# supersimple33/aruco-slam

Measured on AMD Instinct MI355X. Metric: EKF updates/sec at n=1024 landmarks, m=32 obs/frame, higher is better.
Workload: dtype f32 covariance / f64 state

## Files before the change

aruco_slam_amd/_build.py:

```python
from __future__ import annotations

import os
import shutil
import subprocess
from pathlib import Path

PKG = Path(__file__).resolve().parent
CSRC = PKG / "csrc"
LIB_DIR = PKG / "lib"
LIB_PATH = LIB_DIR / "libekf_slam_hip.so"
SOURCES = ["ekf_api.hip", "ekf_batch_api.hip", "ekf_small_kernels.hip", "ekf_front.hip", "ekf_front_f64.hip", "ekf_cov_update.hip", "ekf_cov_macro.hip", "ekf_cov_strip.hip", "ekf_pose_ippe.hip",
           "ekf_wide.hip", "ekf_log.hip", "ekf_gate.hip", "ekf_remove.hip", "ekf_motion.hip", "ekf_batch.hip", "ekf_batch_rot.hip", "ekf_batch_wide.hip", "ekf_batch_moved.hip", "ekf_batch_wide_moved.hip",
           "ekf_batch_frozen.hip", "ekf_batch_wide_frozen.hip",
           "ekf_batch_replicas.hip", "ekf_batch_corner_replicas.hip", "ekf_smooth.hip"]
HEADERS = ["ekf_device.h", "ekf_kernels.h", "ekf_solve_device.h", "ekf_solve_big.h", "ekf_solve_cw.h", "ekf_front_impl.h", "ekf_markers.h", "ekf_host.h", "ekf_batch_impl.h", "ekf_gate_device.h", "ekf_motion_device.h", "ekf_ippe_device.h", "ekf_philox.h", "ekf_remove.h", "ekf_smooth_device.h",
           "../../include/ekf_slam_hip.h"]


def hipcc() -> str:
    for cand in (os.environ.get("HIPCC"), shutil.which("hipcc"), "/opt/rocm/bin/hipcc"):
        if cand and Path(cand).exists():
            return cand
    raise RuntimeError("hipcc not found (need /opt/rocm)")


def _stale(target: Path, deps) -> bool:
    if not target.exists():
        return True
    t = target.stat().st_mtime
    return any(Path(d).stat().st_mtime > t for d in deps)


def build(force: bool = False, verbose: bool = False) -> Path:
    LIB_DIR.mkdir(exist_ok=True)
    obj_dir = PKG / "build"
    obj_dir.mkdir(exist_ok=True)
    hdrs = [CSRC / h for h in HEADERS]
    objs = []
    flags = ["--offload-arch=gfx950", "-O3", "-fPIC", "-std=c++17", "-Wall", "-Wno-unused-function"]
    jobs = []
    for src in SOURCES:
        obj = obj_dir / (Path(src).stem + ".o")
        if force or _stale(obj, [CSRC / src, *hdrs]):
            jobs.append([hipcc(), *flags, "-c", str(CSRC / src), "-o", str(obj)])
        objs.append(obj)
    if jobs:
        from concurrent.futures import ThreadPoolExecutor
        def run(cmd):
            if verbose:
                print(" ".join(cmd))
            subprocess.run(cmd, check=True)
        with ThreadPoolExecutor(max_workers=min(6, len(jobs))) as pool:
            list(pool.map(run, jobs))
    if force or _stale(LIB_PATH, objs):
        cmd = [hipcc(), "--offload-arch=gfx950", "-shared", "-fPIC", "-o", str(LIB_PATH),
               *map(str, objs)]
        if verbose:
            print(" ".join(cmd))
        subprocess.run(cmd, check=True)
    return LIB_PATH


if __name__ == "__main__":
    print(build(verbose=True))
```

aruco_slam_amd/csrc/ekf_api.hip:

```cpp
#include <atomic>
#include <cmath>
#include <cstring>

#include "ekf_host.h"
#include "ekf_kernels.h"
#include "ekf_remove.h"

thread_local std::string g_err;

namespace {

std::atomic<ekf_filter*> g_pipelining{nullptr};

void release_pipelining_token(ekf_filter* f) { (void)g_pipelining.compare_exchange_strong(f, nullptr); }

constexpr int kStageSlots = 64;
constexpr int kMacroSuper = 8;
constexpr int kMacroMinTiles = 3000;
constexpr int kTimedKernels = 4;
constexpr int kWideVisible = 1024;
inline int visible_cap(int model) { return model == EKF_MODEL_ROTATIONS ? 50 : 64; }
inline bool wide_frame(int model, int m) { return m > visible_cap(model); }
constexpr int kEventPool = 2048;

// ... 57 lines not shown
        const size_t nb = (size_t)L.kmax / EKF_RB;
        L.xl_dop = nb * (nb - 1) / 2 * 256 + 64;
        L.xl_y = L.xl_dop + nb * 256;
        L.xl_jac = L.xl_y + L.kmax;
        L.xl_tag = L.xl_jac + (size_t)L.kmax * EKF_JLD;
        L.xl_xs = L.xl_tag + 32;
        L.xl_xr = L.xl_xs + nb * (nb + 1) / 2 * 256;
        L.xl_stag = L.xl_xr + (size_t)round_up(L.kmax, 16);
        L.xl_len = L.xl_stag + 256;
        L.off_xl = w.take(2 * L.xl_len * 8);
        L.off_done = w.take(256);
        L.off_sync = w.take(EKF_SYNC_WORDS * 8);
        L.wsup_ld = (int)round_up(EKF_CAM + (int64_t)L.lmd * c.max_visible, 32);
        L.off_wsup = w.take((size_t)2 * L.kmax * L.wsup_ld * L.elem);
    }
    {
        const int tmax = (int)(L.cap / 128);
        L.tiles_cap = (L.elem == 4 && c.cov_kernel != EKF_COVK_VALU && c.cov_kernel != EKF_COVK_MFMA_TILE)
                          ? tmax * (tmax + 1) / 2 + 8 * kMacroSuper * kMacroSuper : 0;
        L.off_tiles = w.take((size_t)L.tiles_cap * 4);
    }
    L.off_wwork = wide ? w.take((size_t)L.kmax * L.cap * 8) : 0;
    L.off_xinv = wide ? w.take((size_t)EKF_WIDE_BLOCK * EKF_WIDE_BLOCK * 8) : 0;
    L.has_gate = (c.flags & EKF_FLAG_GATE) != 0;
    L.off_gidx = L.has_gate ? w.take((size_t)c.max_visible * 4) : 0;
    L.off_gz = L.has_gate ? w.take((size_t)c.max_visible * 7 * 8) : 0;
    L.off_gmahal = L.has_gate ? w.take((size_t)c.max_visible * 8) : 0;
    L.has_rows = (c.flags & EKF_FLAG_ROW_NOISE) != 0;
    L.off_grow = L.has_rows && L.has_gate ? w.take((size_t)c.max_visible * L.rd * 8) : 0;
    L.total = w.end;
    const size_t det_bytes = align256((size_t)c.max_visible * 4) + align256((size_t)c.max_visible * 56);
    L.slot_exempt = det_bytes;
    L.slot_mahal = det_bytes + align256((size_t)c.max_visible);
    L.slot_rows = L.has_gate ? L.slot_mahal + align256((size_t)c.max_visible * 8) : det_bytes;
    L.slot_bytes = std::max(L.has_rows ? L.slot_rows + align256((size_t)c.max_visible * L.rd * 8) : L.slot_rows,
                            align256(256 * 48) + align256(256 * 80));
    return L;
}

int check_config(const ekf_config* c) {
    if (!c) return fail(EKF_ERR_INVALID, "config is NULL");
    if (c->max_landmarks < 1) return fail(EKF_ERR_INVALID, "max_landmarks must be >= 1");
    if (c->model != EKF_MODEL_EKF && c->model != EKF_MODEL_ROTATIONS)
        return fail(EKF_ERR_INVALID, "unknown model");
    if (c->max_visible < 1 || c->max_visible > ((c->flags & EKF_FLAG_WIDE_FRAMES) ? kWideVisible : visible_cap(c->model)))
        return fail(EKF_ERR_INVALID, (c->flags & EKF_FLAG_WIDE_FRAMES)
                                         ? "max_visible must be in 1..1024 (EKF_FLAG_WIDE_FRAMES)"
                                         : "max_visible must be in 1..64 (1..50 for EKF_MODEL_ROTATIONS; up to 1024 with "
                                           "EKF_FLAG_WIDE_FRAMES)");
    if (c->cov_dtype != EKF_COV_F64 && c->cov_dtype != EKF_COV_F32)
        return fail(EKF_ERR_INVALID, "cov_dtype must be EKF_COV_F64 or EKF_COV_F32");
    if (c->quat_mode != EKF_QUAT_AS_WRITTEN && c->quat_mode != EKF_QUAT_SCALAR_FIRST)
        return fail(EKF_ERR_INVALID, "unknown quat_mode");
    if (c->cov_kernel < EKF_COVK_AUTO || c->cov_kernel > EKF_COVK_MFMA_MACRO)
        return fail(EKF_ERR_INVALID, "unknown cov_kernel");
    if (c->cov_kernel == EKF_COVK_MFMA_MACRO && c->cov_dtype != EKF_COV_F32)
        return fail(EKF_ERR_INVALID, "EKF_COVK_MFMA_MACRO exists for the f32 covariance only");
    if (!(c->r_uncertainty > 0.0)) return fail(EKF_ERR_INVALID, "r_uncertainty must be > 0");
    return EKF_OK;
}

}

struct GetterShortcut {
    bool front_pending = false, mirror_fresh = false, mirror_trust = false, status_clean = false;
    bool zero_copy() const { return mirror_fresh && mirror_trust && status_clean; }
    void frame(bool recorded, bool mirrored) { front_pending = recorded; mirror_fresh = mirrored; }
    void run() { front_pending = status_clean = false; }
    void log() { front_pending = mirror_fresh = false; }
    void markers_added() { front_pending = false; }
    void state_set() { front_pending = mirror_trust = false; }
    void reset() { *this = {false, false, true, true}; }
    void new_workspace() { *this = {}; }
    void removed() { front_pending = mirror_fresh = false; mirror_trust = true; }
    void moved() { front_pending = mirror_fresh = false; }
    void read_back(bool clean, bool full_state) { status_clean = clean; mirror_trust = mirror_trust || full_state; }
};

struct ekf_filter {
    ekf_config cfg{};
    Layout lay{};
    hipStream_t stream = nullptr;
    hipStream_t big = nullptr;
    hipEvent_t ev_front = nullptr;
    GetterShortcut shortcut;
    int device = 0;
    void* cov = nullptr;
    int64_t ld = 0;
    double* state = nullptr;
    char* ws = nullptr;
    bool bound = false, is_reset = false;
    int n_lm = 0;
    int last_m = 0;
    bool debug_w = false;
    bool debug_stamps = false;
    bool debug_stamps_light = false;
    uint64_t fseq = 0;
    uint64_t done_total = 0;
    uint64_t la_base = 0;
    int la_ok = -1;
    int seq_mode = EKF_SEQ_NONE;
    int tiles_T = -1, tiles_grid = 0;
    PinnedBuffer ring, readback, tiles_host;
    int slot = 0;
    hipEvent_t slot_done[kStageSlots] = {};
    bool timing = false;
    bool timing_cov_only = false;
    std::vector<hipEvent_t> ev;
    int ev_frames = 0;
    double t_sum_us[kTimedKernels] = {};
    int64_t t_cnt[kTimedKernels] = {};
    PinnedBuffer log_pin[2];
    hipEvent_t log_pin_done[2] = {};
    int log_pin_turn = 0;
    int64_t log_stats[4] = {};
    double gate = __builtin_inf();
    PinnedBuffer gate_pin;
    hipEvent_t ev_gate = nullptr;
    int64_t gate_stats[2] = {};
    PinnedBuffer remove_pin[2];
    hipEvent_t remove_done[2] = {};
    int remove_turn = 0;

    double pending = 0.0;

    bool frozen = false;

    struct HistoryRec {
        int32_t frame, dims;
        size_t off;
        double s_eff;
        double u[6];
        int32_t stepped, moved;
    };
    struct History {
        bool valid = false;
        const void* buf = nullptr;
        size_t bytes = 0;
        int32_t frames = 0;
        std::vector<HistoryRec> recs;
        std::vector<int32_t> frame_rec;
        std::vector<EkfSmoothRec> table;
    } hist;

    bool has_scale() const { return (cfg.flags & EKF_FLAG_FRAME_SCALE) != 0; }
    bool has_motion() const { return (cfg.flags & EKF_FLAG_MOTION) != 0; }
    bool gate_on() const { return lay.has_gate && gate < __builtin_inf(); }
    void reset_gate_stats() { gate_stats[0] = gate_stats[1] = 0; }
    int dims() const { return lay.lmd * n_lm + EKF_CAM; }
    template <typename P> P* at(size_t off) const { return reinterpret_cast<P*>(ws + off); }
};

namespace {

template <class F>
auto by_cov_type(const ekf_filter* f, F&& fn) {
    return f->lay.elem == 4 ? fn(float{}) : fn(double{});
}

int fold_timing(ekf_filter* f) {
    if (f->ev_frames == 0) return EKF_OK;
    HIP_TRY(hipStreamSynchronize(f->stream));
    for (int fr = 0; fr < f->ev_frames; ++fr) {
        for (int kq = f->timing_cov_only ? kTimedKernels - 1 : 0; kq < kTimedKernels; ++kq) {
            float ms = 0.f;
            HIP_TRY(hipEventElapsedTime(&ms, f->ev[fr * (kTimedKernels + 1) + kq],
                                        f->ev[fr * (kTimedKernels + 1) + kq + 1]));
            f->t_sum_us[kq] += 1e3 * ms;
            f->t_cnt[kq] += 1;
        }
    }
    f->ev_frames = 0;
    return EKF_OK;
}

EkfNoise frame_noise(const ekf_filter* f, double s_eff) {
    return EkfNoise{s_eff * f->cfg.q_cam, s_eff * f->cfg.q_err, s_eff * f->cfg.q_lm, f->cfg.r_uncertainty};
}

bool scale_ok(double s) { return std::isfinite(s) && s >= 0.0; }

EkfFrame make_frame(ekf_filter* f, const int32_t* idx_dev, const double* z_dev, const double* rows_dev, int m,
                    double* traj_row, double s_eff) {
    EkfFrame fr{};
// ... 4 lines not shown
    fr.model = f->cfg.model;
    fr.dims = f->dims();
    fr.ncols = (int)round_up(fr.dims, 128);
    fr.m = m;
    fr.k = L.rd * m;
    fr.kpad = (int)round_up(fr.k, EKF_RB);
    fr.idx = idx_dev;
    fr.z = z_dev;
    fr.rrow = rows_dev;
    fr.jac = f->at<double>(L.off_jac);
    fr.resid = f->at<double>(L.off_resid);
    fr.lmcol = f->at<int32_t>(L.off_lmcol);
    fr.amat = f->at<double>(L.off_amat);
    fr.lda = L.cap;
    fr.sblk = f->at<double>(L.off_sblk);
    fr.lmat = f->at<double>(L.off_lmat);
    fr.ldl = L.kmax;
    fr.dinv = f->at<double>(L.off_dinv);
    fr.lop = f->at<double>(L.off_lop);
    fr.dop = f->at<double>(L.off_dop);
    fr.yvec = f->at<double>(L.off_y);
    fr.wpanel = f->at<void>(L.off_wpanel);
    fr.ldw = L.cap;
    fr.wdbg = f->debug_w ? f->at<double>(L.off_wdbg) : nullptr;
    fr.status = f->at<int32_t>(L.off_status);
    fr.traj_row = traj_row;
    fr.dxvec = f->at<double>(L.off_dx);
    fr.stamps = (f->debug_w || f->debug_stamps) ? f->at<long long>(L.off_stamps) : nullptr;
    fr.stamps_heavy = f->debug_stamps_light ? 0 : 1;
    fr.gate_log = (fr.stamps && !fr.stamps_heavy && !f->debug_w && (size_t)L.kmax * L.cap >= 4 * EKF_GATE_LOG_FRAMES)
                      ? f->at<long long>(L.off_wdbg) : nullptr;
    fr.nz = frame_noise(f, s_eff);
    fr.qprev_cam = fr.nz.q_cam;
    fr.qprev_err = fr.nz.q_err;
    fr.qprev_lm = fr.nz.q_lm;
    fr.quat_mode = f->cfg.quat_mode;
    fr.n_lm = f->n_lm;
    fr.state_host = nullptr;
    fr.status_host = nullptr;
    fr.frozen = f->frozen ? 1 : 0;
    fr.cov_tiles = nullptr;
    fr.cov_grid = 0;
    if (f->tiles_T > 0 && f->tiles_T == (fr.dims + 127) / 128) {
        fr.cov_tiles = f->at<uint32_t>(L.off_tiles);
        fr.cov_grid = f->tiles_grid;
    }
    return fr;
}

bool use_front_kernel(const ekf_filter* f, const EkfFrame& fr) { return (f->cfg.flags & 4) == 0 && fr.kpad <= 192; }

void bind_exchange(ekf_filter* f, EkfFrame& fr) {
    const Layout& L = f->lay;
    double* base = f->at<double>(L.off_xl);
    fr.xl = base + (f->fseq & 1) * L.xl_len;
    fr.xl_next = base + ((f->fseq + 1) & 1) * L.xl_len;
    fr.xl_dop = (int32_t)L.xl_dop;
    fr.xl_y = (int32_t)L.xl_y;
    fr.xl_jac = (int32_t)L.xl_jac;
    fr.xl_tag = (int32_t)L.xl_tag;
    fr.xl_len = (int32_t)L.xl_len;
    fr.xs = fr.xl + L.xl_xs;
    fr.xr = fr.xl + L.xl_xr;
    fr.xs_tag = fr.xl + L.xl_stag;
    fr.seqno = (double)(f->fseq + 1);
    fr.done_ctr = f->at<unsigned long long>(L.off_done);
    f->done_total += (uint64_t)(fr.ncols / 64);
    fr.done_target = f->done_total;
    f->fseq++;
}

int ensure_tiles(ekf_filter* f) {
    const Layout& L = f->lay;
    const int T = (f->dims() + 127) / 128;
    const bool want = L.tiles_cap > 0 &&
                      (f->cfg.cov_kernel == EKF_COVK_MFMA_MACRO || T * (T + 1) / 2 >= kMacroMinTiles);
    if (!want) {
        f->tiles_T = -1;
        return EKF_OK;
    }
    if (f->tiles_T == T) return EKF_OK;
    HIP_TRY(hipStreamSynchronize(f->stream));
    HIP_TRY(hipStreamSynchronize(f->big));
    const int grid = ekf_cov_macro_table(T, kMacroSuper, f->tiles_host.at<uint32_t>(0), L.tiles_cap);
    if (grid <= 0) return fail(EKF_ERR_STATE, "macro-tile launch table does not fit the workspace");
    HIP_TRY(hipMemcpy(f->at<uint32_t>(L.off_tiles), f->tiles_host.get(), (size_t)grid * 4, hipMemcpyHostToDevice));
    f->tiles_T = T;
    f->tiles_grid = grid;
    return EKF_OK;
}

int enqueue_frame(ekf_filter* f, const int32_t* idx_dev, const double* z_dev, const double* rows_dev, int m,
                  double* traj_row, bool mirror, double s_eff) {
    if (!f->frozen) {
        int trc = ensure_tiles(f);
        if (trc) return trc;
    }
    EkfFrame fr = make_frame(f, idx_dev, z_dev, rows_dev, m, traj_row, s_eff);
    const int variant = f->cfg.cov_kernel == EKF_COVK_VALU ? 1 : 2;
    hipEvent_t* ev = nullptr;
    if (f->timing) {
        if (f->ev_frames == kEventPool) {
            int rc = fold_timing(f);
            if (rc) return rc;
        }
        ev = &f->ev[f->ev_frames * (kTimedKernels + 1)];
        f->ev_frames++;
    }
    hipEvent_t* ev_all = (ev && !f->timing_cov_only) ? ev : nullptr;
    if (ev_all) HIP_TRY(hipEventRecord(ev[0], f->stream));
    const bool mirrored = use_front_kernel(f, fr) && !f->timing && mirror && !f->frozen;
    if (use_front_kernel(f, fr)) {
        bind_exchange(f, fr);
        if (mirrored) {
            fr.state_host = f->readback.at<double>(256);
            fr.status_host = f->readback.at<int32_t>(128);
        }
        by_cov_type(f, [&](auto elem) { ekf_launch_front<decltype(elem)>(fr, f->stream); });
        if (ev_all) {
            HIP_TRY(hipEventRecord(ev[1], f->stream));
            HIP_TRY(hipEventRecord(ev[2], f->stream));
        }
    } else if (wide_frame(fr.model, m)) {
        const bool blocked = fr.kpad > EKF_WIDE_REUSE_ROWS;
        const int rp = blocked ? (int)round_up(fr.k, EKF_WIDE_BLOCK) : fr.kpad;
        double* aw = blocked ? f->at<double>(f->lay.off_wwork) : nullptr;
        if (blocked && !f->lay.off_wwork) return fail(EKF_ERR_STATE, "internal: no wide-frame workspace");
        by_cov_type(f, [&](auto elem) { ekf_launch_wide_front<decltype(elem)>(fr, aw, rp, f->stream); });
        if (ev_all) HIP_TRY(hipEventRecord(ev[1], f->stream));
        if (blocked) ekf_launch_wide_factor(fr, aw, f->at<double>(f->lay.off_xinv), rp, f->stream);
        else ekf_launch_solve(fr, f->stream);
        if (ev_all) HIP_TRY(hipEventRecord(ev[2], f->stream));
        by_cov_type(f, [&](auto elem) {
            if (blocked) ekf_launch_wide_finish<decltype(elem)>(fr, aw, f->stream);
            else ekf_launch_panel<decltype(elem)>(fr, f->stream);
        });
        if (fr.model == 1) ekf_launch_inject_rot(fr, f->frozen ? 0 : f->n_lm, f->stream);
    } else {
        by_cov_type(f, [&](auto elem) { ekf_launch_gather<decltype(elem)>(fr, f->stream); });
        if (ev_all) HIP_TRY(hipEventRecord(ev[1], f->stream));
        ekf_launch_solve(fr, f->stream);
        if (ev_all) HIP_TRY(hipEventRecord(ev[2], f->stream));
        by_cov_type(f, [&](auto elem) { ekf_launch_panel<decltype(elem)>(fr, f->stream); });
        if (fr.model == 1) ekf_launch_inject_rot(fr, f->frozen ? 0 : f->n_lm, f->stream);
    }
    f->shortcut.frame(!f->timing && hipEventRecord(f->ev_front, f->stream) == hipSuccess, mirrored);
    if (fr.kpad > EKF_WIDE_REUSE_ROWS) {
        if (ev) HIP_TRY(hipEventRecord(ev[3], f->stream));
        for (int r0 = 0; r0 < fr.kpad; r0 += EKF_WIDE_REUSE_ROWS) {
            EkfFrame cf = fr;
            cf.wpanel = static_cast<char*>(fr.wpanel) + (size_t)r0 * fr.ldw * f->lay.elem;
            cf.kpad = std::min(EKF_WIDE_REUSE_ROWS, fr.kpad - r0);
            cf.k = std::min(cf.kpad, std::max(0, fr.k - r0));
            if (r0 > 0) cf.nz.q_cam = cf.nz.q_err = cf.nz.q_lm = 0.0;
            const bool ok = by_cov_type(f, [&](auto elem) {
                if (f->frozen) return ekf_launch_cov_strip<decltype(elem)>(cf, variant, f->stream);
                ekf_launch_cov_update<decltype(elem)>(cf, variant, f->stream);
                return true;
            });
            if (!ok) return fail(EKF_ERR_STATE, "internal: a row chunk larger than the strip kernel takes");
        }
        if (ev) HIP_TRY(hipEventRecord(ev[4], f->stream));
    } else {
        const bool ok = by_cov_type(f, [&](auto elem) {
            if (f->frozen) return ekf_launch_cov_strip<decltype(elem)>(fr, variant, f->stream, ev ? ev[3] : nullptr, ev ? ev[4] : nullptr);
            ekf_launch_cov_update<decltype(elem)>(fr, variant, f->stream, ev ? ev[3] : nullptr, ev ? ev[4] : nullptr);
            return true;
        });
        if (!ok) return fail(EKF_ERR_STATE, "internal: more rows than the strip kernel takes in one launch");
    }
    HIP_TRY(hipGetLastError());
    f->last_m = m;
    return EKF_OK;
}

int check_ready(ekf_filter* f) {
    if (!f) return fail(EKF_ERR_INVALID, "filter handle is NULL");
    if (!f->bound) return fail(EKF_ERR_STATE, "ekf_bind_buffers has not been called");
    if (!f->is_reset) return fail(EKF_ERR_STATE, "ekf_reset has not been called");
    HIP_TRY(hipSetDevice(f->device));
    return EKF_OK;
}

int sync_and_check(ekf_filter* f, int state_count = 0) {
    if (state_count > 0 && f->shortcut.front_pending) {
        HIP_TRY(hipEventSynchronize(f->ev_front));
        if (f->shortcut.zero_copy() && *f->readback.at<volatile int32_t>(128) == 0)
            return EKF_OK;
        HIP_TRY(hipMemcpyAsync(f->readback.get(), f->at<int32_t>(f->lay.off_status), 32, hipMemcpyDeviceToHost, f->big));
        HIP_TRY(hipMemcpyAsync(f->readback.at<double>(256), f->state, (size_t)state_count * 8, hipMemcpyDeviceToHost, f->big));
        HIP_TRY(hipStreamSynchronize(f->big));
    } else {
        HIP_TRY(hipMemcpyAsync(f->readback.get(), f->at<int32_t>(f->lay.off_status), 32, hipMemcpyDeviceToHost, f->stream));
        if (state_count > 0)
            HIP_TRY(hipMemcpyAsync(f->readback.at<double>(256), f->state, (size_t)state_count * 8, hipMemcpyDeviceToHost, f->stream));
        HIP_TRY(hipStreamSynchronize(f->stream));
        release_pipelining_token(f);
    }
    const int32_t* info = f->readback.at<int32_t>(0);
    const int32_t st = info[0];
    f->shortcut.read_back(st == 0, state_count == f->dims());
    if (st != 0) {
        if (st & EKF_ST_BAD_INDEX)
            return fail(EKF_ERR_INVALID, "landmark index out of range in a device-resident detection array "
                                         "(clamped on the device; the filter state is no longer meaningful, reset it)");
        if (st & (EKF_ST_STALE_JAC | EKF_ST_STALE_COL | EKF_ST_STALE_S))
            return fail(EKF_ERR_NUMERIC, "internal: exchange data of another frame accepted in the front kernel (status " +
                                             std::to_string(st) + ")");
        if (st & EKF_ST_GATE_TIMEOUT)
            return fail(EKF_ERR_NUMERIC, "internal: a device-side wait between the two streams of the pipelined sequence mode timed out");
        if (st & EKF_ST_TIMEOUT)
            return fail(EKF_ERR_NUMERIC, "internal: exchange wait timed out in the front kernel (status " +
                                             std::to_string(st) + ")");
        if (info[2] >= 200)
            return fail(EKF_ERR_NUMERIC, "internal: a wait inside the factorisation workgroup timed out (flag word " +
                                             std::to_string(info[2] - 200) + ")");
        return fail(EKF_ERR_NUMERIC, "innovation covariance S was not positive definite (block column " +
                                         std::to_string(info[2] - 100) + ", wave mask " + std::to_string(info[1]) + ")");
    }
    return EKF_OK;
}

bool pipeline_wanted(const ekf_filter* f, int dims, int kpad, int m) {
    const bool auto_on = !(dims > 9000 && kpad > 96) && !(f->cfg.model == EKF_MODEL_ROTATIONS && kpad > 64);
    const bool want = (f->cfg.flags & 2) != 0 || ((f->cfg.flags & 1) == 0 && auto_on);
    return want && f->lay.has_cov2 && !f->timing && (f->cfg.flags & 4) == 0 && kpad <= 192 &&
           !wide_frame(f->cfg.model, m);
}

int probe_queues(ekf_filter* f) {
    if (f->la_ok >= 0) return EKF_OK;
    unsigned long long* probe = f->at<unsigned long long>(f->lay.off_sync) + 2;
    int32_t* pstat = f->at<int32_t>(f->lay.off_sync) + 8;
    std::vector<hipStream_t> failed;
    auto attempt = [&](bool fresh_stream) {
        if (fresh_stream) {
            hipStream_t fresh = nullptr;
            HIP_TRY(hipStreamCreateWithFlags(&fresh, hipStreamNonBlocking));
            failed.push_back(f->big);
            f->big = fresh;
        }
        HIP_TRY(hipMemsetAsync(probe, 0, 64, f->stream));
        HIP_TRY(hipStreamSynchronize(f->stream));
        ekf_launch_gate(probe, 1ull, pstat, f->big, 1 << 14);
        ekf_launch_signal(probe, 1ull, f->stream);
        HIP_TRY(hipStreamSynchronize(f->big));
        HIP_TRY(hipStreamSynchronize(f->stream));
        int32_t ps = 0;
        HIP_TRY(hipMemcpy(&ps, pstat, 4, hipMemcpyDeviceToHost));
        f->la_ok = (ps == 0) ? 1 : 0;
        return (int)EKF_OK;
    };
    f->la_ok = 0;
    int rc = EKF_OK;
    for (int i = 0; i < 16 && f->la_ok == 0 && rc == EKF_OK; ++i) rc = attempt(i > 0);
    for (hipStream_t s : failed) {
        (void)hipStreamSynchronize(s);
        (void)hipStreamDestroy(s);
    }
    return rc;
}

bool take_pipelining_token(ekf_filter* f) {
    ekf_filter* owner = nullptr;
    if (!g_pipelining.compare_exchange_strong(owner, f) && owner != f) {
        bool idle = hipStreamQuery(owner->stream) == hipSuccess && hipStreamQuery(owner->big) == hipSuccess;
        (void)hipGetLastError();
        if (!(idle && g_pipelining.compare_exchange_strong(owner, f))) return false;
    }
    return true;
}

int choose_pipelining(ekf_filter* f, bool want_runs, int* mode) {
    *mode = EKF_SEQ_SERIAL;
    if (!want_runs || f->frozen) return EKF_OK;
    int rc = probe_queues(f);
    if (rc) return rc;
    if (f->la_ok == 0) *mode = EKF_SEQ_SERIAL_ONE_QUEUE;
    else if (!take_pipelining_token(f)) *mode = EKF_SEQ_SERIAL_OTHER_HANDLE;
    else *mode = EKF_SEQ_PIPELINED;
    return EKF_OK;
}

struct RunFrame {
    const int32_t* idx;
    const double* z;
    int m;
    double* traj_row;
    const double* rows = nullptr;
    double s_eff = 1.0;
};

template <class FrameAt>
int run_pipelined(ekf_filter* f, int frames, FrameAt frame_at, void* other) {
    const Layout& L = f->lay;
    int rc = ensure_tiles(f);
    if (rc) return rc;
    void* wbuf[2] = {f->at<void>(L.off_wpanel), f->at<void>(L.off_wpanel2)};
    void* cbuf[2] = {f->cov, other};
    char* wsup0 = f->at<char>(L.off_wsup);
    void* wsup[2] = {wsup0, wsup0 + (size_t)L.kmax * L.wsup_ld * L.elem};
    unsigned long long* sync = f->at<unsigned long long>(L.off_sync);
    int32_t* status = f->at<int32_t>(L.off_status);
    const uint64_t base = f->la_base;
    f->shortcut.run();
    RunFrame nx = frame_at(0);
    EkfNoise nz_before{};
    for (int t = 0; t < frames; ++t) {
        const int par = t & 1;
        const RunFrame cf_t = nx;
        EkfFrame fr = make_frame(f, cf_t.idx, cf_t.z, cf_t.rows, cf_t.m, cf_t.traj_row, cf_t.s_eff);
        fr.cov = cbuf[0];
        fr.wpanel = wbuf[par];
        if (t > 0) {
            fr.qprev_cam = nz_before.q_cam;
            fr.qprev_err = nz_before.q_err;
            fr.qprev_lm = nz_before.q_lm;
            fr.cov = cbuf[par ^ 1];
            fr.wprev = wbuf[par ^ 1];
            fr.wsup_prev = wsup[par ^ 1];
        }
        const int nb = fr.kpad / EKF_RB;
        const int grid = nb * (nb + 1) / 2 + 2 + fr.ncols / 64;
        fr.wsup_ld = L.wsup_ld;
        fr.la_sync = sync;
        fr.la_signal = (t > 0) ? base + (uint64_t)t : 0;
        fr.la_gate = (t > 0) ? base + (uint64_t)t : 0;
        fr.lds_min = grid <= 100 ? 148 * 1024 : 0;
        if (t + 1 < frames) {
            nx = frame_at(t + 1);
            fr.next_idx = nx.idx;
            fr.next_m = nx.m;
            fr.wsup = wsup[par];
        }
        bind_exchange(f, fr);
        by_cov_type(f, [&](auto elem) { ekf_launch_front<decltype(elem)>(fr, f->stream); });
        EkfFrame cu = fr;
        cu.cov = cbuf[par];
        cu.cov_out = cbuf[par ^ 1];
        if (t + 1 < frames) {
            ekf_launch_gate(sync, base + (uint64_t)t + 1, status, f->big);
            cu.cov_signal = base + (uint64_t)t + 1;
            by_cov_type(f, [&](auto elem) { ekf_launch_cov_update<decltype(elem)>(cu, 2, f->big); });
        } else {
            by_cov_type(f, [&](auto elem) { ekf_launch_cov_update<decltype(elem)>(cu, 2, f->stream); });
        }
        HIP_TRY(hipGetLastError());
        f->last_m = cf_t.m;
        nz_before = fr.nz;
    }
    f->cov = cbuf[frames & 1];
    f->la_base = base + (uint64_t)frames;
    return EKF_OK;
}

struct RunPlan {
    std::vector<char> candidate;
    std::vector<char> joins;
    bool want_runs = false;
};

template <class MOf, class NNewOf>
RunPlan plan_runs(const ekf_filter* f, int frames, MOf m_of, NNewOf nnew_of) {
    RunPlan p;
    p.candidate.assign((size_t)frames, 0);
    p.joins.assign((size_t)frames, 0);
    int prev_kpad = -1;
    int nn = f->n_lm;
    for (int t = 0; t < frames; ++t) {
        const int m = m_of(t);
        if (m == 0) continue;
        const int nnew = nnew_of(t);
        nn += nnew;
        const int kpad = (int)round_up(f->lay.rd * m, EKF_RB);
        p.candidate[t] = pipeline_wanted(f, f->lay.lmd * nn + EKF_CAM, kpad, m);
        p.joins[t] = p.candidate[t] && nnew == 0 && prev_kpad == kpad;
        p.want_runs = p.want_runs || p.joins[t];
        prev_kpad = p.candidate[t] ? kpad : -1;
    }
    return p;
}

template <class FrameOf, class FirstSightings>
int run_frames(ekf_filter* f, int frames, FrameOf frame_of, FirstSightings first_sightings, const RunPlan& plan, bool pipe_ok,
               int64_t* stats) {
    void* const home = f->cov;
    void* const spare = f->lay.has_cov2 ? f->at<void>(f->lay.off_cov2) : nullptr;
    std::vector<int> run;
    auto serial = [&](int t) {
        const RunFrame r = frame_of(t);
        if (stats) stats[0] += 1;
        return enqueue_frame(f, r.idx, r.z, r.rows, r.m, r.traj_row, false, r.s_eff);
    };
    auto flush = [&]() -> int {
        int rc = EKF_OK;
        if (run.size() == 1) {
            rc = serial(run[0]);
        } else if (run.size() >= 2) {
            rc = run_pipelined(f, (int)run.size(), [&](int i) { return frame_of(run[i]); }, f->cov == home ? spare : home);
            if (stats) {
                stats[0] += (int64_t)run.size();
                stats[1] += (int64_t)run.size();
                stats[2] += 1;
            }
        }
        run.clear();
        return rc;
    };
    int rc = EKF_OK;
    for (int t = 0; t < frames && rc == EKF_OK; ++t) {
        if (frame_of(t).m == 0) continue;
        const bool in_run = pipe_ok && plan.candidate[t];
        if (!(in_run && plan.joins[t])) {
            rc = flush();
            if (rc) break;
        }
        const int nnew = first_sightings(t);
        f->n_lm += nnew;
        if (stats) stats[3] += nnew;
        if (in_run) run.push_back(t);
        else rc = serial(t);
    }
    if (rc == EKF_OK) rc = flush();
    if (f->cov != home) {
        hipError_t e = hipMemcpyAsync(home, f->cov, (size_t)f->lay.cap * f->lay.cap * f->lay.elem, hipMemcpyDeviceToDevice,
                                      f->stream);
        f->cov = home;
// ... 175 lines not shown
}

int clear_buffers(const ekf_filter* f, void* cov, double* state, char* ws, const Layout& L) {
    HIP_TRY(hipMemsetAsync(cov, 0, (size_t)L.cap * L.cap * L.elem, f->stream));
    HIP_TRY(hipMemsetAsync(state, 0, (size_t)L.cap * 8, f->stream));
    HIP_TRY(hipMemsetAsync(ws, 0, L.total, f->stream));
    HIP_TRY(hipMemsetD32Async(reinterpret_cast<hipDeviceptr_t>(ws + L.off_xl), (int)0xFFFBADC0u, L.xl_len * 4, f->stream));
    return EKF_OK;
}

void restart_workspace(ekf_filter* f) {
    f->fseq = 0;
    f->done_total = 0;
    f->la_base = 0;
    f->tiles_T = -1;
    std::memset(f->readback.get(), 0, 256 + (size_t)f->lay.cap * 8);
}

}

extern "C" {

const char* ekf_last_error_string(void) { return g_err.c_str(); }

int ekf_default_config(ekf_config* cfg) {
    if (!cfg) return fail(EKF_ERR_INVALID, "config is NULL");
    std::memset(cfg, 0, sizeof(*cfg));
    cfg->max_landmarks = 50;
    cfg->max_visible = 50;
    cfg->cov_dtype = EKF_COV_F64;
    cfg->quat_mode = EKF_QUAT_AS_WRITTEN;
    cfg->cov_kernel = EKF_COVK_AUTO;
    cfg->model = EKF_MODEL_EKF;
    cfg->initial_camera_uncertainty = 0.1;
    cfg->initial_landmark_uncertainty = 0.7;
    cfg->r_uncertainty = 0.9;
    cfg->q_cam = 0.3;
    cfg->q_err = 0.5;
    cfg->q_lm = 0.01;
    cfg->stream = nullptr;
    return EKF_OK;
}

int ekf_query_sizes(const ekf_config* cfg, int64_t* ld, size_t* cov_bytes, size_t* state_bytes,
                    size_t* workspace_bytes) {
    int rc = check_config(cfg);
    if (rc) return rc;
    Layout L = make_layout(*cfg);
    if (ld) *ld = L.cap;
    if (cov_bytes) *cov_bytes = (size_t)L.cap * L.cap * L.elem;
    if (state_bytes) *state_bytes = (size_t)L.cap * 8;
    if (workspace_bytes) *workspace_bytes = L.total;
    return EKF_OK;
}

int ekf_create(const ekf_config* cfg, ekf_filter** out) {
    int rc = check_config(cfg);
    if (rc) return rc;
    if (!out) return fail(EKF_ERR_INVALID, "out is NULL");
    int ndev = 0;
    HIP_TRY(hipGetDeviceCount(&ndev));
    if (ndev < 1) return fail(EKF_ERR_HIP, "no HIP device visible");
    ekf_filter* f = new ekf_filter();
    if (hipGetDevice(&f->device) != hipSuccess) f->device = 0;
    f->cfg = *cfg;
    f->lay = make_layout(*cfg);
    f->stream = static_cast<hipStream_t>(cfg->stream);
    rc = open_handle(f);
    if (rc) {
        ekf_destroy(f);
        return rc;
    }
    *out = f;
    return EKF_OK;
}

int ekf_destroy(ekf_filter* f) {
    if (!f) return EKF_OK;
    (void)hipStreamSynchronize(f->stream);
    if (f->big) {
        (void)hipStreamSynchronize(f->big);
        (void)hipStreamDestroy(f->big);
    }
    release_pipelining_token(f);
    if (f->ev_front) (void)hipEventDestroy(f->ev_front);
    if (f->ev_gate) (void)hipEventDestroy(f->ev_gate);
    for (auto& e : f->remove_done)
        if (e) (void)hipEventDestroy(e);
    for (auto& e : f->ev) (void)hipEventDestroy(e);
    for (int i = 0; i < kStageSlots; ++i)
        if (f->slot_done[i]) (void)hipEventDestroy(f->slot_done[i]);
    for (auto& e : f->log_pin_done)
        if (e) (void)hipEventDestroy(e);
    delete f;
    return EKF_OK;
}

int ekf_bind_buffers(ekf_filter* f, void* cov_dev, int64_t ld, double* state_dev, void* workspace_dev,
                     size_t workspace_bytes) {
    if (!f) return fail(EKF_ERR_INVALID, "filter handle is NULL");
    int rc = check_device_buffers({cov_dev, state_dev, workspace_dev}, workspace_bytes, f->lay.total, "ekf_query_sizes");
    if (rc) return rc;
    if (ld != f->lay.cap) return fail(EKF_ERR_INVALID, "ld must equal the value from ekf_query_sizes");
    f->cov = cov_dev;
    f->ld = ld;
    f->state = state_dev;
    f->ws = static_cast<char*>(workspace_dev);
    f->bound = true;
    f->is_reset = false;
    f->tiles_T = -1;
    return EKF_OK;
}

int ekf_grow(ekf_filter* f, int32_t new_max_landmarks, int32_t new_max_visible, void* cov_dev, int64_t ld, double* state_dev,
             void* workspace_dev, size_t workspace_bytes) {
    if (!f) return fail(EKF_ERR_INVALID, "filter handle is NULL");
    if (!f->bound || !f->is_reset) return fail(EKF_ERR_STATE, "ekf_grow needs a bound, reset filter");
    if (new_max_landmarks < f->cfg.max_landmarks || new_max_visible < f->cfg.max_visible)
        return fail(EKF_ERR_INVALID, "ekf_grow cannot shrink the capacity");
    ekf_config ncfg = f->cfg;
    ncfg.max_landmarks = new_max_landmarks;
    ncfg.max_visible = new_max_visible;
    int rc = check_config(&ncfg);
    if (rc) return rc;
    const Layout nl = make_layout(ncfg);
    rc = check_device_buffers({cov_dev, state_dev, workspace_dev}, workspace_bytes, nl.total,
                              "ekf_query_sizes for the new capacity");
    if (rc) return rc;
    if (ld != nl.cap) return fail(EKF_ERR_INVALID, "ld must equal the value from ekf_query_sizes for the new capacity");
    if (cov_dev == f->cov || state_dev == f->state || workspace_dev == static_cast<void*>(f->ws))
        return fail(EKF_ERR_INVALID, "ekf_grow needs NEW buffers (the old ones are read)");
    HIP_TRY(hipSetDevice(f->device));
    HIP_TRY(hipStreamSynchronize(f->stream));
    HIP_TRY(hipStreamSynchronize(f->big));
    release_pipelining_token(f);
    const Layout& ol = f->lay;
    char* nws = static_cast<char*>(workspace_dev);
    rc = clear_buffers(f, cov_dev, state_dev, nws, nl);
    if (rc) return rc;
    HIP_TRY(hipMemcpyAsync(state_dev, f->state, (size_t)ol.cap * 8, hipMemcpyDeviceToDevice, f->stream));
    HIP_TRY(hipMemcpy2DAsync(cov_dev, (size_t)nl.cap * nl.elem, f->cov, (size_t)ol.cap * ol.elem, (size_t)ol.cap * ol.elem,
                             (size_t)ol.cap, hipMemcpyDeviceToDevice, f->stream));
    HIP_TRY(hipMemcpyAsync(nws + nl.off_status, f->ws + ol.off_status, 32, hipMemcpyDeviceToDevice, f->stream));
    HIP_TRY(hipStreamSynchronize(f->stream));
    rc = reserve_host_buffers(f, nl);
    if (rc) return rc;
    f->cfg = ncfg;
    f->lay = nl;
    f->cov = cov_dev;
    f->ld = ld;
    f->state = state_dev;
    f->ws = nws;
    restart_workspace(f);
    f->shortcut.new_workspace();
    return EKF_OK;
}

int ekf_remove_workspace_bytes(const ekf_filter* f, int32_t count, size_t* bytes) {
    if (!f) return fail(EKF_ERR_INVALID, "filter handle is NULL");
    if (!bytes || count < 0) return fail(EKF_ERR_INVALID, "bad removal size request");
    *bytes = align256((size_t)f->lay.cap * 4);
    return EKF_OK;
}

int ekf_remove_markers(ekf_filter* f, const int32_t* lm_index, int32_t count, void* cov_dev_new, int64_t ld,
                       double* state_dev_new, void* remove_ws, size_t remove_ws_bytes) {
    int rc = check_ready(f);
    if (rc) return rc;
    if (count < 0 || (count > 0 && !lm_index)) return fail(EKF_ERR_INVALID, "bad removal list");
    const Layout& L = f->lay;
    const size_t need = align256((size_t)L.cap * 4);
    rc = check_device_buffers({cov_dev_new, state_dev_new, remove_ws}, need, need, "ekf_remove_workspace_bytes");
    if (rc) return rc;
    if (ld != L.cap) return fail(EKF_ERR_INVALID, "ld must equal the value from ekf_query_sizes");
    if (cov_dev_new == f->cov || state_dev_new == f->state)
        return fail(EKF_ERR_INVALID, "ekf_remove_markers needs NEW buffers (the old ones are read)");
    if (remove_ws_bytes < need) return fail(EKF_ERR_CAPACITY, "remove_ws smaller than ekf_remove_workspace_bytes");
    std::vector<int32_t> sorted;
    const std::string bad = ekf_remove_build_map(lm_index, count, f->n_lm, L.lmd, L.cap, nullptr, sorted);
    if (!bad.empty()) return fail(EKF_ERR_INVALID, bad);
    if (count == 0) return EKF_OK;
    const int turn = f->remove_turn;
    PinnedBuffer& pin = f->remove_pin[turn];
    hipEvent_t& done = f->remove_done[turn];
    if ((rc = pin.reserve(need))) return rc;
    if (!done) HIP_TRY(hipEventCreateWithFlags(&done, hipEventDisableTiming));
    HIP_TRY(hipEventSynchronize(done));
    (void)ekf_remove_build_map(lm_index, count, f->n_lm, L.lmd, L.cap, pin.at<int32_t>(0), sorted);
    HIP_TRY(hipMemcpyAsync(remove_ws, pin.get(), (size_t)L.cap * 4, hipMemcpyHostToDevice, f->stream));
    HIP_TRY(hipEventRecord(done, f->stream));
    f->remove_turn = turn ^ 1;
    const int64_t n_old = f->dims(), n_new = n_old - (int64_t)L.lmd * count;
    EkfRemoveArgs a{};
    a.cov_src = f->cov;
    a.cov_dst = cov_dev_new;
    a.state_src = f->state;
    a.state_dst = state_dev_new;
    a.ld = L.cap;
    a.map = static_cast<const int32_t*>(remove_ws);
    a.state_host = f->readback.at<double>(256);
    a.n_new = (int32_t)n_new;
    if (L.has_cov2) {
        a.cov2 = f->at<void>(L.off_cov2);
        a.fringe_hi = (int32_t)std::min<int64_t>(round_up(n_old, 128), L.cap);
    }
    by_cov_type(f, [&](auto elem) { ekf_launch_remove<decltype(elem)>(a, 1, f->stream); });
    HIP_TRY(hipGetLastError());
    f->shortcut.removed();
    f->hist.valid = false;
    f->cov = cov_dev_new;
    f->state = state_dev_new;
    f->n_lm -= count;
    return EKF_OK;
}

int ekf_reset(ekf_filter* f, const double initial_camera_pose[10]) {
    if (!f) return fail(EKF_ERR_INVALID, "filter handle is NULL");
    if (!f->bound) return fail(EKF_ERR_STATE, "ekf_bind_buffers has not been called");
    if (!initial_camera_pose) return fail(EKF_ERR_INVALID, "initial pose is NULL");
    HIP_TRY(hipSetDevice(f->device));
    const Layout& L = f->lay;
    HIP_TRY(hipStreamSynchronize(f->stream));
    int rc = clear_buffers(f, f->cov, f->state, f->ws, L);
    if (rc) return rc;
    restart_workspace(f);
    f->shortcut.reset();
    HIP_TRY(hipMemcpyAsync(f->state, initial_camera_pose, 10 * sizeof(double), hipMemcpyHostToDevice,
                           f->stream));
    char diag[8 * EKF_CAM];
    by_cov_type(f, [&](auto elem) {
        for (int i = 0; i < EKF_CAM; ++i)
            reinterpret_cast<decltype(elem)*>(diag)[i] = (decltype(elem))f->cfg.initial_camera_uncertainty;
    });
    HIP_TRY(hipMemcpy2DAsync(f->cov, (size_t)(L.cap + 1) * L.elem, diag, L.elem, L.elem, EKF_CAM,
                             hipMemcpyHostToDevice, f->stream));
    HIP_TRY(hipStreamSynchronize(f->stream));
    f->n_lm = 0;
    f->last_m = 0;
    f->pending = 0.0;
    f->frozen = false;
    f->hist.valid = false;
    f->is_reset = true;
    return EKF_OK;
}

int ekf_add_markers(ekf_filter* f, const double* cam_frame_xyz, const double* diag_uncertainty,
                    int32_t count) {
    int rc = check_ready(f);
    if (rc) return rc;
    if (count < 0 || (count > 0 && !cam_frame_xyz)) return fail(EKF_ERR_INVALID, "bad marker list");
    if (f->n_lm + count > f->cfg.max_landmarks)
        return fail(EKF_ERR_CAPACITY, "more landmarks than max_landmarks");
    const Layout& L = f->lay;
    f->shortcut.markers_added();
    int done = 0;
    while (done < count) {
        const int chunk = std::min(256, count - done);
        char* slot = f->ring.get() + (size_t)f->slot * L.slot_bytes;
        HIP_TRY(hipEventSynchronize(f->slot_done[f->slot]));
        double* hx = reinterpret_cast<double*>(slot);
        double* hu = reinterpret_cast<double*>(slot + align256(256 * 48));
        const bool rot = f->cfg.model == EKF_MODEL_ROTATIONS;
        const size_t pb = rot ? 48 : 24, ub = rot ? 80 : 24;
        std::memcpy(hx, cam_frame_xyz + (pb / 8) * done, (size_t)chunk * pb);
        if (diag_uncertainty) std::memcpy(hu, diag_uncertainty + (ub / 8) * done, (size_t)chunk * ub);
        HIP_TRY(hipMemcpyAsync(f->at<double>(L.off_xyz), hx, (size_t)chunk * pb, hipMemcpyHostToDevice,
                               f->stream));
        if (diag_uncertainty)
            HIP_TRY(hipMemcpyAsync(f->at<double>(L.off_unc), hu, (size_t)chunk * ub,
                                   hipMemcpyHostToDevice, f->stream));
        const double* unc_dev = diag_uncertainty ? f->at<double>(L.off_unc) : nullptr;
        by_cov_type(f, [&](auto elem) {
            auto* launch = rot ? ekf_launch_add_markers_rot<decltype(elem)> : ekf_launch_add_markers<decltype(elem)>;
            launch(f->cov, f->ld, f->state, f->dims(), f->at<double>(L.off_xyz), unc_dev, f->cfg.initial_landmark_uncertainty,
                   chunk, f->stream);
        });
        HIP_TRY(hipGetLastError());
        HIP_TRY(hipEventRecord(f->slot_done[f->slot], f->stream));
        f->slot = (f->slot + 1) % kStageSlots;
        f->n_lm += chunk;
        done += chunk;
    }
    return EKF_OK;
}

int ekf_observe(ekf_filter* f, const int32_t* lm_index, const double* z, int32_t m) {
    int rc = check_ready(f);
    if (rc) return rc;
    f->reset_gate_stats();
    return observe_host(f, lm_index, z, nullptr, m, f->gate_on(), nullptr, nullptr, nullptr);
}

int ekf_observe_gated(ekf_filter* f, const int32_t* lm_index, const double* z, int32_t m, const uint8_t* exempt, double* mahal,
                      int32_t* survivors) {
    int rc = check_ready(f);
    if (rc) return rc;
    if (!f->lay.has_gate) return fail(EKF_ERR_STATE, "the filter was created without EKF_FLAG_GATE");
    f->reset_gate_stats();
    const bool gated = f->gate_on() || mahal;
    rc = observe_host(f, lm_index, z, nullptr, m, gated, exempt, mahal, survivors);
    if (rc == EKF_OK && !gated && survivors) *survivors = m;
    return rc;
}

namespace {
// ... 42 lines not shown
    if ((rc = check_scales(f, &scale, 1))) return rc;
    f->pending = f->pending + scale;
    return EKF_OK;
}

int ekf_get_pending_scale(const ekf_filter* f, double* out) {
    if (!f) return fail(EKF_ERR_INVALID, "filter handle is NULL");
    if (!out) return fail(EKF_ERR_INVALID, "out is NULL");
    *out = f->pending;
    return EKF_OK;
}

int ekf_set_pending_scale(ekf_filter* f, double pending) {
    int rc = check_ready(f);
    if (rc) return rc;
    if ((rc = check_scales(f, &pending, 1))) return rc;
    f->pending = pending;
    return EKF_OK;
}

int ekf_set_gate(ekf_filter* f, double gate) {
    if (!f) return fail(EKF_ERR_INVALID, "filter handle is NULL");
    if (!f->lay.has_gate) return fail(EKF_ERR_STATE, "the filter was created without EKF_FLAG_GATE");
    if (!(gate > 0.0)) return fail(EKF_ERR_INVALID, "the gate must be > 0 (+inf: off) and not NaN");
    f->gate = gate;
    return EKF_OK;
}

int ekf_last_gate_stats(const ekf_filter* f, int64_t out[2]) {
    if (!f) return fail(EKF_ERR_INVALID, "filter handle is NULL");
    if (!out) return fail(EKF_ERR_INVALID, "out is NULL");
    out[0] = f->gate_stats[0];
    out[1] = f->gate_stats[1];
    return EKF_OK;
}

int ekf_observe_device(ekf_filter* f, const int32_t* lm_index_dev, const double* z_dev, int32_t m) {
    int rc = check_ready(f);
    if (rc) return rc;
    if (m < 1) return fail(EKF_ERR_INVALID, "observe needs at least one detection");
    if (m > f->cfg.max_visible) return fail(EKF_ERR_CAPACITY, "more detections than max_visible");
    if (!lm_index_dev || !z_dev) return fail(EKF_ERR_INVALID, "NULL detections");
    if (f->n_lm < 1) return fail(EKF_ERR_STATE, "observe before any landmark was added");
    f->reset_gate_stats();
    const double s_eff = frame_scale(f, nullptr);
    int s = m;
    rc = f->gate_on() ? gated_frame(f, lm_index_dev, z_dev, nullptr, m, nullptr, 0, nullptr, nullptr, nullptr, true, &s, s_eff)
                      : enqueue_frame(f, lm_index_dev, z_dev, nullptr, m, nullptr, true, s_eff);
    if (rc == EKF_OK) frame_scale_done(f, nullptr, s_eff, s > 0);
    return rc;
}

int ekf_observe_sequence_device(ekf_filter* f, const int32_t* lm_index_dev, const double* z_dev,
                                int32_t m, int32_t frames, double* trajectory_dev) {
    return ekf_observe_sequence_device_rows(f, lm_index_dev, z_dev, nullptr, m, frames, trajectory_dev);
}

int ekf_observe_sequence_device_rows(ekf_filter* f, const int32_t* lm_index_dev, const double* z_dev, const double* rows_dev,
                                     int32_t m, int32_t frames, double* trajectory_dev) {
    return ekf_observe_sequence_device_scaled(f, lm_index_dev, z_dev, rows_dev, nullptr, m, frames, trajectory_dev);
}

int ekf_observe_sequence_device_scaled(ekf_filter* f, const int32_t* lm_index_dev, const double* z_dev, const double* rows_dev,
                                       const double* scale, int32_t m, int32_t frames, double* trajectory_dev) {
    return ekf_observe_sequence_device_moved(f, lm_index_dev, z_dev, rows_dev, scale, nullptr, m, frames, trajectory_dev);
}

int ekf_observe_sequence_device_moved(ekf_filter* f, const int32_t* lm_index_dev, const double* z_dev, const double* rows_dev,
                                      const double* scale, const double* motion, int32_t m, int32_t frames,
                                      double* trajectory_dev) {
    int rc = check_ready(f);
    if (rc) return rc;
    if (rows_dev && !f->lay.has_rows) return fail(EKF_ERR_STATE, "the filter was created without EKF_FLAG_ROW_NOISE");
    if (m < 1 || frames < 0) return fail(EKF_ERR_INVALID, "bad sequence shape");
    if ((rc = check_scales(f, scale, frames))) return rc;
    if ((rc = check_motions(f, motion, frames))) return rc;
    if (m > f->cfg.max_visible) return fail(EKF_ERR_CAPACITY, "more detections than max_visible");
    if (!lm_index_dev || !z_dev) return fail(EKF_ERR_INVALID, "NULL detections");
    if (f->n_lm < 1) return fail(EKF_ERR_STATE, "observe before any landmark was added");
    const int rd = f->lay.rd;
    f->reset_gate_stats();
    if (f->gate_on() || motion || f->frozen) {
        f->seq_mode = EKF_SEQ_SERIAL;
        f->shortcut.log();
        for (int t = 0; t < frames; ++t) {
            int s = m;
            const double* sc = scale ? scale + t : nullptr;
            if ((rc = enqueue_motion(f, motion ? motion + (size_t)t * 6 : nullptr))) return rc;
            const double s_eff = frame_scale(f, sc);
            const int32_t* idx_t = lm_index_dev + (size_t)t * m;
            const double* z_t = z_dev + (size_t)t * m * rd;
            const double* rows_t = rows_dev ? rows_dev + (size_t)t * m * rd : nullptr;
            double* row_t = trajectory_dev ? trajectory_dev + (size_t)t * 7 : nullptr;
            rc = f->gate_on() ? gated_frame_or_row(f, idx_t, z_t, rows_t, m, nullptr, 0, nullptr, row_t, &s, s_eff)
                              : enqueue_frame(f, idx_t, z_t, rows_t, m, row_t, false, s_eff);
            if (rc) return rc;
            frame_scale_done(f, sc, s_eff, s > 0);
        }
        f->shortcut.log();
        return EKF_OK;
    }
    std::vector<double> s_effs((size_t)frames, 1.0);
    for (int t = 0; t < frames; ++t) {
        s_effs[t] = frame_scale(f, scale ? scale + t : nullptr);
        frame_scale_done(f, scale ? scale + t : nullptr, s_effs[t], true);
    }
    const RunPlan plan = plan_runs(f, frames, [&](int) { return m; }, [](int) { return 0; });
    int mode = EKF_SEQ_SERIAL;
    rc = choose_pipelining(f, plan.want_runs, &mode);
    if (rc) return rc;
    f->seq_mode = mode == EKF_SEQ_PIPELINED ? EKF_SEQ_SERIAL : mode;
    rc = run_frames(
        f, frames,
        [&](int t) {
            return RunFrame{lm_index_dev + (size_t)t * m, z_dev + (size_t)t * m * rd, m,
                            trajectory_dev ? trajectory_dev + (size_t)t * 7 : nullptr,
                            rows_dev ? rows_dev + (size_t)t * m * rd : nullptr, s_effs[t]};
        },
        [](int) { return 0; }, plan, mode == EKF_SEQ_PIPELINED, nullptr);
    if (rc) return rc;
    f->seq_mode = mode;
    return EKF_OK;
}

}

namespace {

struct LogLayout {
    size_t idx, slots, total;
};

LogLayout log_layout(int rd, int64_t D) {
    Carve w;
    w.take((size_t)D * rd * 8);
    const size_t idx = w.take((size_t)D * 4), slots = w.take((size_t)D * 4);
    return {idx, slots, std::max<size_t>(256, w.end)};
}

int smoothing_supported(const ekf_filter* f) {
    if (f->cfg.model != EKF_MODEL_EKF) return fail(EKF_ERR_STATE, "smoothing: EKF_MODEL_ROTATIONS is not supported");
    if (f->cfg.cov_dtype != EKF_COV_F64) return fail(EKF_ERR_STATE, "smoothing needs the f64 covariance");
    if (f->cfg.quat_mode != EKF_QUAT_SCALAR_FIRST)
        return fail(EKF_ERR_STATE, "smoothing needs EKF_QUAT_SCALAR_FIRST (the as-written injection has no inverse)");
    if (f->frozen) return fail(EKF_ERR_STATE, "smoothing: the map is frozen");
    return EKF_OK;
}

size_t history_record_bytes(int64_t dims) { return align256((size_t)(dims + dims * (dims + 1) / 2) * 8); }

void history_bound(int lmd, int n_lm, const LogCheck& lc, int64_t frames, size_t* bytes) {
    size_t total = 256;
    for (int64_t t = 0; t < frames; ++t) total += history_record_bytes(EKF_CAM + (int64_t)lmd * (n_lm + lc.new_at[t + 1]));
    *bytes = total;
}

struct SmoothLayout {
    size_t table, xs, xp, yv, wv, cv, xinv, M, total;
};
SmoothLayout smooth_layout(size_t records, int64_t nmax) {
    const size_t npad = (size_t)round_up(std::max<int64_t>(nmax, 1), EKF_WIDE_BLOCK);
    Carve w;
    w.take(256);
    SmoothLayout L{};
    L.table = w.take(std::max<size_t>(records, 1) * sizeof(EkfSmoothRec));
    L.xs = w.take(npad * 8);
// ... 446 lines not shown
    if (rc) return rc;
    if (!out || count < 0 || count > f->dims()) return fail(EKF_ERR_INVALID, "bad state request");
    rc = sync_and_check(f, count);
    if (rc) return rc;
    std::memcpy(out, f->readback.at<double>(256), (size_t)count * 8);
    return EKF_OK;
}

int ekf_get_camera(ekf_filter* f, double out[10]) { return ekf_get_state(f, out, EKF_CAM); }

int ekf_get_cov_diag(ekf_filter* f, double* out, int32_t count) {
    int rc = check_ready(f);
    if (rc) return rc;
    if (!out || count < 0 || count > f->dims()) return fail(EKF_ERR_INVALID, "bad diag request");
    double* scratch = f->at<double>(f->lay.off_diag);
    by_cov_type(f, [&](auto elem) { ekf_launch_cov_diag<decltype(elem)>(f->cov, f->ld, scratch, count, f->stream); });
    HIP_TRY(hipGetLastError());
    rc = sync_and_check(f);
    if (rc) return rc;
    HIP_TRY(hipMemcpy(out, scratch, (size_t)count * 8, hipMemcpyDeviceToHost));
    return EKF_OK;
}

int ekf_get_cov(ekf_filter* f, double* out, int32_t dims) {
    int rc = check_ready(f);
    if (rc) return rc;
    if (!out || dims != f->dims()) return fail(EKF_ERR_INVALID, "dims must equal the state dimension");
    rc = sync_and_check(f);
    if (rc) return rc;
    const size_t el = f->lay.elem;
    if (el == 8) {
        HIP_TRY(hipMemcpy2D(out, (size_t)dims * 8, f->cov, (size_t)f->ld * 8, (size_t)dims * 8, dims,
                            hipMemcpyDeviceToHost));
    } else {
        std::vector<float> tmp((size_t)dims * dims);
        HIP_TRY(hipMemcpy2D(tmp.data(), (size_t)dims * 4, f->cov, (size_t)f->ld * 4, (size_t)dims * 4,
                            dims, hipMemcpyDeviceToHost));
        for (size_t i = 0; i < tmp.size(); ++i) out[i] = (double)tmp[i];
    }
    return EKF_OK;
}

int ekf_set_state(ekf_filter* f, const double* state, int32_t num_landmarks) {
    int rc = check_ready(f);
    if (rc) return rc;
    if (!state || num_landmarks < 0) return fail(EKF_ERR_INVALID, "bad state");
    if (num_landmarks > f->cfg.max_landmarks)
        return fail(EKF_ERR_CAPACITY, "more landmarks than max_landmarks");
    f->shortcut.state_set();
    HIP_TRY(hipStreamSynchronize(f->stream));
    HIP_TRY(hipMemset(f->state, 0, (size_t)f->lay.cap * 8));
    HIP_TRY(hipMemcpy(f->state, state, (size_t)(f->lay.lmd * num_landmarks + EKF_CAM) * 8,
                      hipMemcpyHostToDevice));
    f->n_lm = num_landmarks;
    f->pending = 0.0;
    return EKF_OK;
}

int ekf_set_cov(ekf_filter* f, const double* cov, int32_t dims) {
    int rc = check_ready(f);
    if (rc) return rc;
    if (!cov || dims != f->dims())
        return fail(EKF_ERR_INVALID, "dims must equal the state dimension (call ekf_set_state first)");
    const Layout& L = f->lay;
    HIP_TRY(hipStreamSynchronize(f->stream));
    HIP_TRY(hipMemset(f->cov, 0, (size_t)L.cap * L.cap * L.elem));
    if (L.has_cov2) {
        HIP_TRY(hipStreamSynchronize(f->big));
        HIP_TRY(hipMemset(f->at<void>(L.off_cov2), 0, (size_t)L.cap * L.cap * L.elem));
    }
    return by_cov_type(f, [&](auto elem) -> int {
        using T = decltype(elem);
        std::vector<T> tmp((size_t)dims * dims);
        for (int i = 0; i < dims; ++i)
            for (int j = 0; j < dims; ++j)
                tmp[(size_t)i * dims + j] = (T)(0.5 * (cov[(size_t)i * dims + j] + cov[(size_t)j * dims + i]));
        HIP_TRY(hipMemcpy2D(f->cov, (size_t)f->ld * sizeof(T), tmp.data(), (size_t)dims * sizeof(T), (size_t)dims * sizeof(T),
                            dims, hipMemcpyHostToDevice));
        return EKF_OK;
    });
}

int ekf_last_sequence_mode(const ekf_filter* f) { return f ? f->seq_mode : EKF_ERR_INVALID; }

int ekf_set_map_frozen(ekf_filter* f, int32_t frozen) {
    int rc = check_ready(f);
    if (rc) return rc;
    f->frozen = frozen != 0;
    return EKF_OK;
}

int ekf_get_map_frozen(const ekf_filter* f) { return f ? (f->frozen ? 1 : 0) : EKF_ERR_INVALID; }

int ekf_set_fused(ekf_filter* f, int32_t enable) {
    if (!f) return fail(EKF_ERR_INVALID, "filter handle is NULL");
    if (enable) f->cfg.flags &= ~4; else f->cfg.flags |= 4;
    return EKF_OK;
}

int ekf_set_kernel_timing(ekf_filter* f, int32_t enable) {
    if (!f) return fail(EKF_ERR_INVALID, "filter handle is NULL");
    HIP_TRY(hipStreamSynchronize(f->stream));
    if (enable && f->ev.empty()) {
        f->ev.resize((size_t)kEventPool * (kTimedKernels + 1));
        for (auto& e : f->ev) HIP_TRY(hipEventCreate(&e));
    }
    f->timing = enable != 0;
    f->timing_cov_only = enable == 2;
    f->ev_frames = 0;
    for (int i = 0; i < kTimedKernels; ++i) {
        f->t_sum_us[i] = 0.0;
        f->t_cnt[i] = 0;
    }
    return EKF_OK;
}

int ekf_get_kernel_timing(ekf_filter* f, int32_t which, double* mean_us, int64_t* launches) {
    if (!f) return fail(EKF_ERR_INVALID, "filter handle is NULL");
    if (which < 0 || which >= kTimedKernels) return fail(EKF_ERR_INVALID, "which must be 0..3");
    int rc = fold_timing(f);
    if (rc) return rc;
    if (mean_us) *mean_us = f->t_cnt[which] ? f->t_sum_us[which] / (double)f->t_cnt[which] : 0.0;
    if (launches) *launches = f->t_cnt[which];
    return EKF_OK;
}

int ekf_debug_fetch(ekf_filter* f, int32_t what, double* out, size_t count) {
    int rc = check_ready(f);
    if (rc) return rc;
    if (!out) return fail(EKF_ERR_INVALID, "out is NULL");
    if (what == -1) {
        f->debug_w = true;
        return EKF_OK;
    }
    if (what == -2 || what == -3) {
        f->debug_stamps = true;
        f->debug_stamps_light = what == -3;
        return EKF_OK;
    }
    const Layout& L = f->lay;
    const int k = L.rd * f->last_m, kp = (int)round_up(k, EKF_RB), dims = f->dims();
    const int jc = f->cfg.model == EKF_MODEL_ROTATIONS ? 20 : EKF_JCOLS;
    HIP_TRY(hipStreamSynchronize(f->stream));
    switch (what) {
        case 0:
            if (count < (size_t)k * jc) return fail(EKF_ERR_INVALID, "out too small");
            HIP_TRY(hipMemcpy2D(out, (size_t)jc * 8, f->at<double>(L.off_jac), EKF_JLD * 8, (size_t)jc * 8,
                                k, hipMemcpyDeviceToHost));
            return EKF_OK;
        case 1:
            if (count < (size_t)k) return fail(EKF_ERR_INVALID, "out too small");
            HIP_TRY(hipMemcpy(out, f->at<double>(L.off_resid), (size_t)k * 8, hipMemcpyDeviceToHost));
            return EKF_OK;
        case 2:
            if (count < (size_t)kp * kp) return fail(EKF_ERR_INVALID, "out too small");
            HIP_TRY(hipMemcpy2D(out, (size_t)kp * 8, f->at<double>(L.off_lmat), (size_t)L.kmax * 8,
                                (size_t)kp * 8, kp, hipMemcpyDeviceToHost));
            return EKF_OK;
        case 3:
            if (!f->debug_w) return fail(EKF_ERR_STATE, "call ekf_debug_fetch(f,-1,..) first");
            if (count < (size_t)kp * dims) return fail(EKF_ERR_INVALID, "out too small");
            HIP_TRY(hipMemcpy2D(out, (size_t)dims * 8, f->at<double>(L.off_wdbg), (size_t)L.cap * 8,
                                (size_t)dims * 8, kp, hipMemcpyDeviceToHost));
            return EKF_OK;
        case 4:
            if (count < (size_t)k * dims) return fail(EKF_ERR_INVALID, "out too small");
// ... 28 lines not shown
```

aruco_slam_amd/csrc/ekf_cov_update.hip:

```cpp
#include <hip/hip_ext.h>
#include "ekf_kernels.h"

template <typename T>
__device__ __forceinline__ void ekf_cov_store(T* p, T v) {
    __hip_atomic_store(p, v, __ATOMIC_RELAXED, __HIP_MEMORY_SCOPE_AGENT);
}

typedef float f32x16 __attribute__((ext_vector_type(16)));
typedef double f64x4 __attribute__((ext_vector_type(4)));

template <typename T>
__global__ __launch_bounds__(256) void ekf_cov_update_valu(EkfFrame fr) {
    __shared__ T sa[16][64];
    __shared__ T sb[16][64];
    const int tid = threadIdx.x, tx = tid & 15, ty = tid >> 4;
    const int i0 = blockIdx.y * 64, j0 = blockIdx.x * 64;
    const T* __restrict__ wp = static_cast<const T*>(fr.wpanel);
    T acc[4][4];
#pragma unroll
    for (int x = 0; x < 4; ++x)
#pragma unroll
        for (int y = 0; y < 4; ++y) acc[x][y] = (T)0;
    for (int kc = 0; kc < fr.kpad; kc += 16) {
#pragma unroll
// ... 205 lines not shown
    for (int ri = 0; ri < 2; ++ri)
#pragma unroll
        for (int ci = 0; ci < 2; ++ci)
#pragma unroll
            for (int r = 0; r < 4; ++r) {
                const int rl = 16 * ri + g + 4 * r, cl = 16 * ci + c;
                double v = pt[ri][ci][r];
                if (I == J && rl == cl) v += ekf_qdiag(i0 + rl, fr.dims, fr.nz);
                v += acc[ri][ci][r];
                ekf_cov_store(Pout + (int64_t)(i0 + rl) * ld + j0 + cl, v);
                if (I != J) tr[wave][rl][cl] = v;
            }
    if (I != J) {
        __builtin_amdgcn_wave_barrier();
        const int l31 = lane & 31, lhi = lane >> 5;
#pragma unroll
        for (int it = 0; it < 16; ++it) {
            const int cc = 2 * it + lhi;
            ekf_cov_store(Pout + (int64_t)(j0 + cc) * ld + i0 + l31, tr[wave][l31][cc]);
        }
    }
    if (fr.cov_signal) ekf_cov_arrive(fr);
}

__global__ __launch_bounds__(256) void ekf_cov_update_mfma_f64_split(EkfFrame fr, int nitems) {
    __shared__ double tr[32][33];
    const int wave = threadIdx.x >> 6, lane = threadIdx.x & 63;
    const int c = lane & 15, g = lane >> 4;
    const int ri = wave >> 1, ci = wave & 1;
    int I, J;
    ekf_tri_decode(blockIdx.x, I, J);
    const int i0 = 32 * I, j0 = 32 * J;
    const double* __restrict__ wp = static_cast<const double*>(fr.wpanel);
    const double* P = static_cast<const double*>(fr.cov);
    double* Pout = fr.cov_out ? static_cast<double*>(fr.cov_out) : static_cast<double*>(fr.cov);
    const int64_t ld = fr.ld, ldw = fr.ldw;
    double pt[4];
#pragma unroll
    for (int r = 0; r < 4; ++r) pt[r] = P[(int64_t)(i0 + 16 * ri + g + 4 * r) * ld + j0 + 16 * ci + c];
    f64x4 acc = {0.0, 0.0, 0.0, 0.0};
    const double* wa = wp + (int64_t)g * ldw + i0 + 16 * ri + c;
    const double* wb = wp + (int64_t)g * ldw + j0 + 16 * ci + c;
    const int steps = fr.kpad >> 2;
    for (int ks = 0; ks < steps; ks += 4) {
        double a[4], b[4];
#pragma unroll
        for (int u = 0; u < 4; ++u) {
            const int64_t off = (int64_t)(4 * (ks + u)) * ldw;
            a[u] = wa[off];
            b[u] = wb[off];
        }
#pragma unroll
        for (int u = 0; u < 4; ++u) acc = __builtin_amdgcn_mfma_f64_16x16x4f64(-a[u], b[u], acc, 0, 0, 0);
    }
#pragma unroll
    for (int r = 0; r < 4; ++r) {
        const int rl = 16 * ri + g + 4 * r, cl = 16 * ci + c;
        double v = pt[r];
        if (I == J && rl == cl) v += ekf_qdiag(i0 + rl, fr.dims, fr.nz);
        v += acc[r];
        ekf_cov_store(Pout + (int64_t)(i0 + rl) * ld + j0 + cl, v);
        if (I != J) tr[rl][cl] = v;
    }
    if (I != J) {
        __syncthreads();
        const int l31 = threadIdx.x & 31;
        for (int cc = threadIdx.x >> 5; cc < 32; cc += 8)
            ekf_cov_store(Pout + (int64_t)(j0 + cc) * ld + i0 + l31, tr[l31][cc]);
    }
    if (fr.cov_signal) ekf_cov_arrive(fr);
}

__global__ void ekf_gate_kernel(unsigned long long* counter, unsigned long long target, int32_t* status, int max_polls) {
    if (threadIdx.x != 0) return;
    int it = 0;
    while (__hip_atomic_load(counter, __ATOMIC_RELAXED, __HIP_MEMORY_SCOPE_SYSTEM) < target) {
        if (++it > max_polls) { atomicOr(status, EKF_ST_GATE_TIMEOUT); break; }
        __builtin_amdgcn_s_sleep(8);
    }
}
__global__ void ekf_signal_kernel(unsigned long long* counter, unsigned long long value) {
    if (threadIdx.x == 0) __hip_atomic_store(counter, value, __ATOMIC_RELAXED, __HIP_MEMORY_SCOPE_SYSTEM);
}
void ekf_launch_gate(unsigned long long* counter, unsigned long long target, int32_t* status, hipStream_t s, int max_polls) {
    hipLaunchKernelGGL(ekf_gate_kernel, dim3(1), dim3(64), 0, s, counter, target, status, max_polls);
}
void ekf_launch_signal(unsigned long long* counter, unsigned long long value, hipStream_t s) {
    hipLaunchKernelGGL(ekf_signal_kernel, dim3(1), dim3(64), 0, s, counter, value);
}

#define EKF_COV_LAUNCH(kernel, grid, block, s, e0, e1, ...)                                     \
    do {                                                                                         \
        if (e0) hipExtLaunchKernelGGL(kernel, grid, block, 0, s, e0, e1, 0, __VA_ARGS__);        \
        else hipLaunchKernelGGL(kernel, grid, block, 0, s, __VA_ARGS__);                         \
    } while (0)

static inline int ekf_tri_items(const EkfFrame& fr) {
    const int t = (fr.dims + 31) / 32;
    return t * (t + 1) / 2;
}

template <>
void ekf_launch_cov_update<float>(const EkfFrame& fr, int variant, hipStream_t s, hipEvent_t e0, hipEvent_t e1) {
    if (variant == 1) {
        EKF_COV_LAUNCH(ekf_cov_update_valu<float>, dim3(fr.ncols / 64, fr.ncols / 64), dim3(256), s, e0, e1, fr);
    } else if (fr.cov_tiles) {
        ekf_launch_cov_update_macro(fr, s, e0, e1);
    } else {
        const int items = ekf_tri_items(fr);
        const dim3 grid((items + 3) / 4), block(256);
        switch (fr.kpad / 16) {
#define EKF_COV_CASE(KB) case KB: EKF_COV_LAUNCH((ekf_cov_update_mfma_f32<KB, 3, (KB <= 8) ? 5 : 4>), grid, block, s, e0, e1, fr, items); break;
            EKF_COV_CASE(1) EKF_COV_CASE(2) EKF_COV_CASE(3) EKF_COV_CASE(4) EKF_COV_CASE(5) EKF_COV_CASE(6)
            EKF_COV_CASE(7) EKF_COV_CASE(8) EKF_COV_CASE(9) EKF_COV_CASE(10) EKF_COV_CASE(11) EKF_COV_CASE(12)
            EKF_COV_CASE(13) EKF_COV_CASE(14) EKF_COV_CASE(15) EKF_COV_CASE(16) EKF_COV_CASE(17) EKF_COV_CASE(18)
            EKF_COV_CASE(19) EKF_COV_CASE(20) EKF_COV_CASE(21) EKF_COV_CASE(22) EKF_COV_CASE(23) EKF_COV_CASE(24)
            default: break;
#undef EKF_COV_CASE
        }
    }
}
template <>
void ekf_launch_cov_update<double>(const EkfFrame& fr, int variant, hipStream_t s, hipEvent_t e0, hipEvent_t e1) {
    if (variant == 1) {
        EKF_COV_LAUNCH(ekf_cov_update_valu<double>, dim3(fr.ncols / 64, fr.ncols / 64), dim3(256), s, e0, e1, fr);
    } else {
        const int items = ekf_tri_items(fr);
        if (items <= 2048)
            EKF_COV_LAUNCH(ekf_cov_update_mfma_f64_split, dim3(items), dim3(256), s, e0, e1, fr, items);
        else
            EKF_COV_LAUNCH(ekf_cov_update_mfma_f64, dim3((items + 3) / 4), dim3(256), s, e0, e1, fr, items);
    }
}
```

aruco_slam_amd/csrc/ekf_front_impl.h:

```cpp
#pragma once
#include "ekf_solve_big.h"

#define FR_T 512
#define FR_ALD 66
#define FR_KS 96
#define FR_KS64 48
__host__ __device__ inline size_t fr_chunk_a_len(int kpad, bool fix, int elem) {
    const size_t a = (size_t)kpad * FR_ALD;
    const size_t st = elem == 4 ? (size_t)(FR_KS * 128 + FR_KS * 64 + 128 * 64) / 2 : (size_t)(2 * FR_KS64 * 64 + 64 * 64);
    return (fix && a < st) ? st : a;
}
#define FR_SLOTS 4

typedef double pf64x4 __attribute__((ext_vector_type(4)));
template <typename T>
__device__ __forceinline__ void fr_w_store(T* p, T v) {
    __hip_atomic_store(p, v, __ATOMIC_RELAXED, __HIP_MEMORY_SCOPE_AGENT);
}
typedef float fr_f32x16 __attribute__((ext_vector_type(16)));

__device__ __forceinline__ void ekf_poll_sleep() { __builtin_amdgcn_s_sleep(4); }

template <int MODEL>
__device__ __forceinline__ void fr_measure(const EkfFrame& fr, const double* cam, const int* lmc, double* hs,
                                           double* rsd, int tid, bool publish) {
    constexpr int RD = EkfModel<MODEL>::RD, LMD = EkfModel<MODEL>::LMD, JC = EkfModel<MODEL>::JC;
    if (tid < fr.m) {
        const int c0 = lmc[tid];
        double lm[LMD], h[RD];
        for (int d = 0; d < LMD; ++d) lm[d] = fr.state[c0 + d];
        double (*J)[JC] = reinterpret_cast<double (*)[JC]>(hs + (size_t)RD * tid * JC);
        ekf_measure_model<MODEL>(cam, lm, h, J);
        if (publish) {
            for (int d = 0; d < RD; ++d) {
                for (int a = 0; a < JC; ++a) fr.jac[(size_t)(RD * tid + d) * EKF_JLD + a] = J[d][a];
                const double rv = fr.z[RD * tid + d] - h[d];
                fr.resid[RD * tid + d] = rv;
                rsd[RD * tid + d] = rv;
            }
            fr.lmcol[tid] = c0;
        }
    }
    if (publish)
        for (int r = fr.k + tid; r < fr.kpad; r += FR_T) rsd[r] = 0.0;
}

template <bool QPREV> __device__ __forceinline__ double fr_qdiag_prev(const EkfFrame& fr, int i) {
    if constexpr (QPREV) return ekf_qdiag_prev(fr, i);
    else return ekf_qdiag(i, fr.dims, fr.nz);
}

template <typename T, int MODEL, int NB, bool ROWS, bool QPREV>
__device__ __forceinline__ void fr_role_sblock(const EkfFrame& fr, int sb, int nS, double* sm) {
    constexpr int RD = EkfModel<MODEL>::RD, LMD = EkfModel<MODEL>::LMD, JC = EkfModel<MODEL>::JC;
    constexpr int NSLOT = EKF_CAM + LMD * EkfModel<MODEL>::NDET16;
    double* hs = sm;
    double* us = sm + fr.k * JC;
    int* lmc = reinterpret_cast<int*>(us + NSLOT * 16);
    double* rsd = us + NSLOT * 16 + 32;
    const int tid = threadIdx.x, m = fr.m, k = fr.k;
    const T* __restrict__ P = static_cast<const T*>(fr.cov);
    const int64_t ld = fr.ld;
    double cam[EKF_CAM];
#pragma unroll
    for (int a = 0; a < EKF_CAM; ++a) cam[a] = fr.state[a];
    if (fr.stamps && sb == 0 && tid == 0) fr.stamps[60] = wall_clock64();
    int bi = 0, bj = sb;
    while (bj > bi) { bj -= bi + 1; ++bi; }
    const int j0 = (16 * bi) / RD, jc0 = (16 * bj) / RD;
    [[maybe_unused]] double rnoise = 0.0;
    if constexpr (ROWS && !QPREV) {
        if (bi == bj && tid < 16 && 16 * bi + tid < k) rnoise = fr.rrow[16 * bi + tid];
    } else if constexpr (ROWS) {
        if (bi == bj && tid < 16 && 16 * bi + tid < k) rnoise = fr.rrow ? fr.rrow[16 * bi + tid] : fr.nz.r_unc;
    }
    const bool fix = fr.wsup_prev != nullptr;
    constexpr int NT16 = (NSLOT + 15) / 16, DLD16 = 16 * NT16, DLD64 = DLD16;
    double* dots64 = rsd + fr.kpad;
    float* dots = reinterpret_cast<float*>(rsd + fr.kpad);
    const int dlane = tid & 63, dc = dlane & 15, dg = dlane >> 4, dtile = 7 - (tid >> 6);
    constexpr int KS4 = 4 * NB, KB = KS4 < 24 ? KS4 : 24;
    const bool dotw = sizeof(T) == 4 && fix && dtile < NT16 * NT16;
    const float* __restrict__ wsd = static_cast<const float*>(fr.wsup_prev);
    float oa[KB], ob[KB];
    auto dot_operands = [&](int tile, int s0) {
        const int smax = fr.wsup_ld - 1;
        const int rs = 16 * (tile / NT16) + dc, cs = 16 * (tile % NT16) + dc;
        const int gr = (rs < EKF_CAM) ? rs : min(EKF_CAM + LMD * j0 + (rs - EKF_CAM), smax);
        const int gc = (cs < EKF_CAM) ? cs : min(EKF_CAM + LMD * jc0 + (cs - EKF_CAM), smax);
#pragma unroll
        for (int u = 0; u < KB; ++u)
            if (s0 + u < KS4) {
                const float* kb = wsd + (int64_t)(4 * (s0 + u) + dg) * fr.wsup_ld;
                oa[u] = kb[gr];
                ob[u] = kb[gc];
            }
    };
    if (dotw) dot_operands(dtile, 0);
    if (tid < m) lmc[tid] = ekf_lm_column(fr, LMD, tid, false);
    if constexpr (ROWS)
        if (bi == bj && tid < 16) rsd[tid] = rnoise;
    __syncthreads();
    constexpr int NE = (NSLOT * 16 + FR_T - 1) / FR_T;
    int urho[NE], uc20[NE], ur2[NE];
// ... 69 lines not shown
            if (uact[n]) {
                const int uslot = (tid + FR_T * n) >> 4;
                const int cdet = EKF_CAM + LMD * (ur2[n] / RD - jc0);
#pragma unroll
                for (int b = 0; b < JC; ++b) {
                    const int col = (b < EKF_CAM) ? b : uc20[n] + (b - EKF_CAM);
                    const int cs = (b < EKF_CAM) ? b : cdet + (b - EKF_CAM);
                    if constexpr (sizeof(T) == 4) {
                        const float q = (col == urho[n]) ? (float)fr_qdiag_prev<QPREV>(fr, urho[n]) : 0.0f;
                        pv[n][b] = (T)(((float)pv[n][b] + q) + dots[uslot * DLD16 + cs]);
                    } else {
                        double v = (double)pv[n][b];
                        if (col == urho[n]) v += fr_qdiag_prev<QPREV>(fr, urho[n]);
                        pv[n][b] = (T)(v + dots64[uslot * DLD64 + cs]);
                    }
                }
            }
        }
    }
#pragma unroll
    for (int n = 0; n < NE; ++n) {
        const int ue = tid + FR_T * n;
        if (ue < NSLOT * 16) {
            double acc = 0.0;
            if (uact[n]) {
                const double* h2 = hs + ur2[n] * JC;
#pragma unroll
                for (int b = 0; b < JC; ++b) {
                    const int col = (b < EKF_CAM) ? b : uc20[n] + (b - EKF_CAM);
                    const double pq = (double)pv[n][b] + ((col == urho[n]) ? ekf_qdiag(urho[n], fr.dims, fr.nz) : 0.0);
                    acc = __builtin_fma(pq, h2[b], acc);
                }
            }
            us[ue] = acc;
        }
    }
    __syncthreads();
    double v = 0.0;
    if (tid < 256) {
        const int i = tid >> 4, c2 = tid & 15, r1 = 16 * bi + i, r2 = 16 * bj + c2;
        if (r1 >= k || r2 >= k) {
            v = (r1 == r2) ? 1.0 : 0.0;
        } else if (r2 > r1) {
            v = 0.0;
        } else {
            const double* h1 = hs + r1 * JC;
            const int s1 = EKF_CAM + LMD * (r1 / RD - j0);
            double acc;
            if constexpr (ROWS) acc = (r1 == r2) ? rsd[i] : 0.0;
            else acc = (r1 == r2) ? fr.nz.r_unc : 0.0;
#pragma unroll
            for (int a = 0; a < EKF_CAM; ++a) acc = __builtin_fma(h1[a], us[a * 16 + c2], acc);
#pragma unroll
            for (int d = 0; d < LMD; ++d) acc = __builtin_fma(h1[EKF_CAM + d], us[(s1 + d) * 16 + c2], acc);
            v = acc;
        }
    }
    __syncthreads();
    if (tid < 256) us[(tid >> 4) * 17 + (tid & 15)] = v;
    __syncthreads();
    if (tid < 64) {
        sv_sblock_emit<true>(fr.xs + sv_blk_index(bi, bj), us, bi == bj, tid);
        if (tid == 0) ekf_stc(fr.xs_tag + 16 * bj + bi, fr.seqno);
    }
    if (fr.stamps && sb == nS - 1 && tid == 0) fr.stamps[61] = wall_clock64();

    {
        const int64_t lo = (int64_t)fr.xl_len * sb / nS, hi = (int64_t)fr.xl_len * (sb + 1) / nS;
        const double sent = ekf_sent();
        for (int64_t e = lo + tid; e < hi; e += FR_T) ekf_stc(fr.xl_next + e, sent);
    }
}

template <int MODEL>
__device__ __forceinline__ void fr_role_measure(const EkfFrame& fr, double* sm) {
    constexpr int LMD = EkfModel<MODEL>::LMD, JC = EkfModel<MODEL>::JC;
    double* hs = sm;
    double* rsd = sm + fr.k * JC;
    int* lmc = reinterpret_cast<int*>(rsd + fr.kpad);
    const int tid = threadIdx.x;
    if (fr.stamps && !fr.stamps_heavy && tid == 0) {
        const long long now = wall_clock64();
        fr.stamps[16 + ((long long)fr.seqno & 15)] = now;
        if (fr.gate_log) fr.gate_log[4 * ((long long)fr.seqno & (EKF_GATE_LOG_FRAMES - 1))] = now;
    }
    if (fr.la_signal && tid == 0)
        __hip_atomic_store(fr.la_sync, fr.la_signal, __ATOMIC_RELAXED, __HIP_MEMORY_SCOPE_SYSTEM);
    double cam[EKF_CAM];
#pragma unroll
    for (int a = 0; a < EKF_CAM; ++a) cam[a] = fr.state[a];
    if (tid < fr.m) lmc[tid] = ekf_lm_column(fr, LMD, tid, true);
    __syncthreads();
    fr_measure<MODEL>(fr, cam, lmc, hs, rsd, tid, true);
    __syncthreads();
    double* __restrict__ xj = fr.xl + fr.xl_jac;
    const int nel = fr.k * JC;
    for (int e = tid; e < nel; e += FR_T) ekf_stc(xj + e, hs[e]);
    for (int e = tid; e < fr.kpad; e += FR_T) ekf_stc(fr.xr + e, rsd[e]);
    if (tid == 0) {
        ekf_stc(fr.xl + fr.xl_tag, fr.seqno);
        ekf_stc(fr.xl + fr.xl_tag + 16, fr.seqno);
    }
    if (fr.stamps && tid == 0) fr.stamps[55] = wall_clock64();
    if (fr.la_gate && tid == 0) {
        const long long g0 = fr.gate_log ? wall_clock64() : 0;
        int it = 0;
        while (__hip_atomic_load(fr.la_sync + 1, __ATOMIC_RELAXED, __HIP_MEMORY_SCOPE_SYSTEM) < fr.la_gate) {
            if (++it > (1 << 22)) { ekf_raise(fr, EKF_ST_GATE_TIMEOUT); break; }
            __builtin_amdgcn_s_sleep(8);
        }
        if (fr.gate_log) {
            long long* row = fr.gate_log + 4 * ((long long)fr.seqno & (EKF_GATE_LOG_FRAMES - 1));
            row[1] = g0;
            row[2] = wall_clock64();
            row[3] = it;
        }
    }
}

__device__ __forceinline__ int fr_tag_stale(double tag, double seqno) { return !ekf_is_sent(tag) && tag != seqno; }
struct SvIoFused {
    const EkfFrame& fr;
    int spin_fail, stale;
    __device__ __forceinline__ bool settled(const sf64x4& v) const {
        return !__any(ekf_is_sent(v[0]) || ekf_is_sent(v[1]) || ekf_is_sent(v[2]) || ekf_is_sent(v[3]));
    }
    __device__ __forceinline__ void settle_block(sf64x4& v, int i, int tc, int lane) {
        const double* base = fr.xs + sv_blk_index(i, tc);
        int it = 0;
        while (!settled(v)) {
            if (++it > EKF_SPIN_MAX) { spin_fail = 1; break; }
            ekf_poll_sleep();
            v = sf64x4{ekf_ldc(base + 2 * lane), ekf_ldc(base + 2 * lane + 1), ekf_ldc(base + 128 + 2 * lane),
                       ekf_ldc(base + 129 + 2 * lane)};
        }
    }
    __device__ __forceinline__ sf64x4 fetch_resid(int tc, int g) {
        const double* base = fr.xr + EKF_RB * tc + g;
        sf64x4 v = {ekf_ldc(base), ekf_ldc(base + 4), ekf_ldc(base + 8), ekf_ldc(base + 12)};
        int it = 0;
        while (!settled(v)) {
            if (++it > EKF_SPIN_MAX) { spin_fail = 1; break; }
            ekf_poll_sleep();
            v = sf64x4{ekf_ldc(base), ekf_ldc(base + 4), ekf_ldc(base + 8), ekf_ldc(base + 12)};
        }
        return v;
    }
    template <int NB, int N0, int N1, int C0, int C1>
    __device__ __forceinline__ void load_cols(sf64x4 (&z0)[N0], sf64x4 (&z1)[N1], int i0, int i1, bool has0, bool has1,
                                              int lane, int g) {
        const bool blk0 = has0 && i0 < NB, blk1 = has1 && i1 < NB;
        const bool res0 = C0 == 0 && has0 && i0 == NB, res1 = C0 == 0 && has1 && i1 == NB;
        const int r0 = blk0 ? i0 : 0, r1 = blk1 ? i1 : r0;
        double t0[N0], t1[N1];
#pragma unroll
        for (int tc = C0; tc < N0 && tc < C1; ++tc) t0[tc] = ekf_ldc(fr.xs_tag + 16 * min(tc, r0) + r0);
#pragma unroll
        for (int tc = C0; tc < N1 && tc < C1; ++tc) t1[tc] = ekf_ldc(fr.xs_tag + 16 * min(tc, r1) + r1);
#pragma unroll
        for (int tc = C0; tc < N0 && tc < C1; ++tc) {
            const double* p0 = fr.xs + sv_blk_index(r0, min(tc, r0)) + 2 * lane;
            if (!(has0 && i0 == NB)) z0[tc] = sf64x4{ekf_ldc(p0), ekf_ldc(p0 + 1), ekf_ldc(p0 + 128), ekf_ldc(p0 + 129)};
        }
#pragma unroll
        for (int tc = C0; tc < N1 && tc < C1; ++tc) {
            const double* p0 = fr.xs + sv_blk_index(r1, min(tc, r1)) + 2 * lane;
            if (!(has1 && i1 == NB)) z1[tc] = sf64x4{ekf_ldc(p0), ekf_ldc(p0 + 1), ekf_ldc(p0 + 128), ekf_ldc(p0 + 129)};
        }
#pragma unroll
        for (int tc = C0; tc < N0 && tc < C1; ++tc) {
            stale |= fr_tag_stale(t0[tc], fr.seqno);
            if (blk0 && tc <= i0) settle_block(z0[tc], i0, tc, lane);
        }
#pragma unroll
        for (int tc = C0; tc < N1 && tc < C1; ++tc) {
            stale |= fr_tag_stale(t1[tc], fr.seqno);
            if (blk1 && tc <= i1) settle_block(z1[tc], i1, tc, lane);
        }
        if (res0) {
#pragma unroll
            for (int tc = 0; tc < N0; ++tc)
                if (tc < NB) {
                    const double* base = fr.xr + EKF_RB * tc + g;
                    z0[tc] = sf64x4{ekf_ldc(base), ekf_ldc(base + 4), ekf_ldc(base + 8), ekf_ldc(base + 12)};
                }
#pragma unroll
            for (int tc = 0; tc < N0; ++tc)
                if (tc < NB && !settled(z0[tc])) z0[tc] = fetch_resid(tc, g);
            stale |= fr_tag_stale(ekf_ldc(fr.xl + fr.xl_tag + 16), fr.seqno);
        }
        if (res1) {
#pragma unroll
            for (int tc = 0; tc < N1; ++tc)
                if (tc < NB) {
                    const double* base = fr.xr + EKF_RB * tc + g;
                    z1[tc] = sf64x4{ekf_ldc(base), ekf_ldc(base + 4), ekf_ldc(base + 8), ekf_ldc(base + 12)};
                }
#pragma unroll
            for (int tc = 0; tc < N1; ++tc)
                if (tc < NB && !settled(z1[tc])) z1[tc] = fetch_resid(tc, g);
            stale |= fr_tag_stale(ekf_ldc(fr.xl + fr.xl_tag + 16), fr.seqno);
        }
    }
    __device__ __forceinline__ sf64x4 fetch_block(int i, int tc, int lane) {
        const double* p0 = fr.xs + sv_blk_index(i, tc) + 2 * lane;
        const double tag = ekf_ldc(fr.xs_tag + 16 * tc + i);
        sf64x4 v = {ekf_ldc(p0), ekf_ldc(p0 + 1), ekf_ldc(p0 + 128), ekf_ldc(p0 + 129)};
        stale |= fr_tag_stale(tag, fr.seqno);
        settle_block(v, i, tc, lane);
        return v;
    }
    __device__ __forceinline__ sf64x4 hist_block(int i, int q, int lane) const {
        const double* base = fr.xl + sv_lop_index(i, q) + lane;
        return sf64x4{ekf_ldc(base), ekf_ldc(base + 64), ekf_ldc(base + 128), ekf_ldc(base + 192)};
    }
    __device__ __forceinline__ void put_dinv(int b, const sf64x4& xop, int lane) {
        double* xdop = fr.xl + fr.xl_dop;
#pragma unroll
        for (int r = 0; r < 4; ++r) ekf_stc(xdop + (size_t)(b * 4 + r) * 64 + lane, xop[r]);
        if (lane == 0) ekf_stc(fr.xl + fr.xl_tag + 1 + b, fr.seqno);
    }
    __device__ __forceinline__ void put_l(int i, int b, const sf64x4& y, int lane) {
#pragma unroll
        for (int r = 0; r < 4; ++r) ekf_stc(fr.xl + sv_lop_index(i, b) + r * 64 + lane, -y[r]);
    }
    __device__ __forceinline__ void put_y(int b, double yv, int c, bool active) {
        if (active) ekf_stc(fr.xl + fr.xl_y + EKF_RB * b + c, yv);
    }
};

template <int NB>
__device__ __forceinline__ void fr_role_factor(const EkfFrame& fr, double* v_sm) {
    const int tid = threadIdx.x, lane = tid & 63, wave = tid >> 6;
    if (fr.stamps && tid == 0) fr.stamps[62] = wall_clock64();
    SvIoFused io{fr, 0, 0};
    int bad = 0, badcol = 0;
    sv_factor_any<NB>(fr, io, v_sm, bad, badcol);
    if ((bad | io.spin_fail | io.stale) && lane == 0) {
        ekf_raise(fr, (bad ? EKF_ST_NOT_SPD : 0) | (io.spin_fail ? EKF_ST_TIMEOUT : 0) | (io.stale ? EKF_ST_STALE_S : 0));
        if (bad) {
            atomicOr(fr.status + 1, 1 << wave);
            atomicCAS(fr.status + 2, 0, badcol);
        }
    }
    if (fr.stamps && tid == 0) fr.stamps[63] = wall_clock64();
    if (tid < 256) {
        const int tc = tid >> 4, i = tid & 15;
        if (tc <= i && i < NB && fr_tag_stale(ekf_ldc(fr.xs_tag + 16 * tc + i), fr.seqno)) ekf_raise(fr, EKF_ST_STALE_S);
    }
}

template <int NB>
struct FrPre {
    static constexpr int SLOT = NB * 256 + 16;
    double dqn[4], yqn[4];
    unsigned long long smask;
    int sdim;
    double st_old, q_old[4];
};
template <int NB, int MODEL>
__device__ __forceinline__ void fr_panel_pre(const EkfFrame& fr, FrPre<NB>& pre, const unsigned long long* smask_l, int wv, int col0, int lane) {
    const int j = lane & 15, g = lane >> 4;
    if constexpr (NB == 1) {
#pragma unroll
        for (int r = 0; r < 4; ++r) {
            pre.dqn[r] = (wv == 0) ? ekf_ldc(fr.xl + fr.xl_dop + (size_t)r * 64 + lane) : 0.0;
            pre.yqn[r] = (wv == 0) ? ekf_ldc(fr.xl + fr.xl_y + g + 4 * r) : 0.0;
        }
    }
    const int mycol = col0 + j;
    pre.st_old = 0.0;
#pragma unroll
    for (int i = 0; i < 4; ++i) pre.q_old[i] = 0.0;
    if (MODEL == 0) {
        if (mycol < fr.dims && !(fr.frozen && mycol >= EKF_CAM)) pre.st_old = fr.state[mycol];
        if (col0 == 0)
            for (int i = 0; i < 4; ++i) pre.q_old[i] = fr.state[3 + i];
    }
    pre.smask = fr.wsup ? smask_l[16 * wv + j] : 0ull;
    pre.sdim = (mycol >= EKF_CAM) ? (mycol - EKF_CAM) % EkfModel<MODEL>::LMD : 0;
}

template <int NB>
__device__ __forceinline__ void fr_panel_stage(const EkfFrame& fr, double* slots, volatile ekf_lds_int* flags, int w, int lane) {
    constexpr int SLOT = FrPre<NB>::SLOT;
    constexpr bool HELP = NB <= 8;
    const double* __restrict__ xlop = fr.xl;
    const double* __restrict__ xdop = fr.xl + fr.xl_dop;
    const double* __restrict__ xy = fr.xl + fr.xl_y;
    __syncthreads();
    int spin_fail = 0;
    for (int q = w; q < NB; q += 4) {
        const int cnt = NB - 1 - q;
        const int sl = q % FR_SLOTS;
        double* slot = slots + sl * SLOT;
        double dv[4], yv = 0.0;
        double v[NB - 1][4];
        auto load_dy = [&]() {
#pragma unroll
            for (int r = 0; r < 4; ++r) dv[r] = ekf_ldc(xdop + (size_t)(q * 4 + r) * 64 + lane);
            yv = ekf_ldc(xy + 16 * q + (lane & 15));
        };
        auto pend_dy = [&]() {
            bool pend = ekf_is_sent(yv);
#pragma unroll
            for (int r = 0; r < 4; ++r) pend = pend || ekf_is_sent(dv[r]);
            return __any(pend) != 0;
        };
        auto fetch = [&]() {
#pragma unroll
// ... 187 lines not shown
    } else {
        const double* __restrict__ xdop = fr.xl + fr.xl_dop;
        const double* __restrict__ xy = fr.xl + fr.xl_y;
        double dq[4], yq[4];
        if (wv == 0) {
            bool pend = false;
#pragma unroll
            for (int r = 0; r < 4; ++r) {
                dq[r] = pre.dqn[r];
                yq[r] = pre.yqn[r];
                pend = pend || ekf_is_sent(dq[r]) || ekf_is_sent(yq[r]);
            }
            if (__any(pend)) {
                for (int it = 0;; ++it) {
                    pend = false;
#pragma unroll
                    for (int r = 0; r < 4; ++r) {
                        dq[r] = ekf_ldc(xdop + (size_t)r * 64 + lane);
                        yq[r] = ekf_ldc(xy + g + 4 * r);
                        pend = pend || ekf_is_sent(dq[r]) || ekf_is_sent(yq[r]);
                    }
                    if (!__any(pend)) break;
                    if (it > EKF_SPIN_MAX) { spin_fail = 1; break; }
                    ekf_poll_sleep();
                }
            }
            int it = 0;
            while (sync[1] < 0) {
                if (++it > 64 * EKF_SPIN_MAX) { spin_fail = 1; break; }
                __builtin_amdgcn_s_sleep(1);
            }
            __builtin_amdgcn_fence(__ATOMIC_ACQUIRE, "workgroup");
#pragma unroll
            for (int r = 0; r < 4; ++r) {
                pshare[r * 64 + lane] = dq[r];
                pshare[(4 + r) * 64 + lane] = yq[r];
            }
            __builtin_amdgcn_fence(__ATOMIC_RELEASE, "workgroup");
            if (lane == 0) sync[0] = 1;
        } else {
            int it = 0;
            while (sync[0] < 1) {
                if (++it > 64 * EKF_SPIN_MAX) { spin_fail = 1; break; }
                __builtin_amdgcn_s_sleep(1);
            }
            __builtin_amdgcn_fence(__ATOMIC_ACQUIRE, "workgroup");
#pragma unroll
            for (int r = 0; r < 4; ++r) {
                dq[r] = pshare[r * 64 + lane];
                yq[r] = pshare[(4 + r) * 64 + lane];
            }
            __builtin_amdgcn_fence(__ATOMIC_RELEASE, "workgroup");
            if (lane == 0) __hip_atomic_fetch_add(const_cast<ekf_lds_int*>(sync) + 1, 1, __ATOMIC_RELAXED, __HIP_MEMORY_SCOPE_WORKGROUP);
        }
        pf64x4 wq = {0.0, 0.0, 0.0, 0.0};
#pragma unroll
        for (int r = 0; r < 4; ++r) wq = __builtin_amdgcn_mfma_f64_16x16x4f64(dq[r], t[0][r], wq, 0, 0, 0);
        t[0] = wq;
#pragma unroll
        for (int r = 0; r < 4; ++r) {
            const int row = g + 4 * r;
            fr_w_store(wp + (int64_t)row * fr.ldw + col0 + j, (T)wq[r]);
            if (fr.wdbg) fr.wdbg[(int64_t)row * fr.ldw + col0 + j] = wq[r];
            if (cslot >= 0) fr_w_store(wsup + (int64_t)row * fr.wsup_ld + cslot, (T)wq[r]);
            for (unsigned long long mm = smask; mm; mm &= mm - 1) {
                constexpr int LMD = EkfModel<MODEL>::LMD;
                const int jj = __builtin_ctzll(mm);
                fr_w_store(wsup + (int64_t)row * fr.wsup_ld + EKF_CAM + LMD * jj + sdim, (T)wq[r]);
            }
        }
#pragma unroll
        for (int r = 0; r < 4; ++r) part = __builtin_fma(wq[r], yq[r], part);
        if (stp) stp[0] = wall_clock64();
    }
    part += __shfl_xor(part, 16);
    part += __shfl_xor(part, 32);
    const int col = col0 + j;
    if (MODEL == 1) {
        if (g == 0) ekf_stc(fr.dxvec + col, part);
    } else {
        double nv = 0.0;
        if (g == 0 && (col < 3 || (col >= EKF_CAM && col < fr.dims && !fr.frozen))) {
            nv = st_old + part;
            fr.state[col] = nv;
            if (fr.state_host) fr.state_host[col] = nv;
        }
        if (col0 == 0) {
            const double e0 = __shfl(part, 7), e1 = __shfl(part, 8), e2 = __shfl(part, 9);
            const double x0 = __shfl(nv, 0), x1 = __shfl(nv, 1), x2 = __shfl(nv, 2);
            if (lane == 0) {
                double qv[4] = {q_old[0], q_old[1], q_old[2], q_old[3]};
                const double err[3] = {e0, e1, e2};
                ekf_quat_inject_n(qv, q_rn, err, fr.quat_mode);
                for (int i = 0; i < 4; ++i) fr.state[3 + i] = qv[i];
                for (int i = 0; i < 3; ++i) fr.state[7 + i] = 0.0;
                if (fr.state_host) {
                    for (int i = 0; i < 4; ++i) fr.state_host[3 + i] = qv[i];
                    for (int i = 0; i < 3; ++i) fr.state_host[7 + i] = 0.0;
                }
                if (fr.traj_row) {
                    fr.traj_row[0] = x0; fr.traj_row[1] = x1; fr.traj_row[2] = x2;
                    for (int i = 0; i < 4; ++i) fr.traj_row[3 + i] = qv[i];
                }
            }
        }
    }
    if (stp) stp[NB] = wall_clock64();
    if (wv == 0 && lane < NB && fr_tag_stale(ekf_ldc(fr.xl + fr.xl_tag + 1 + lane), fr.seqno)) ekf_raise(fr, EKF_ST_STALE_COL);
    if (wv == 0 && lane == NB && fr_tag_stale(ekf_ldc(fr.xl + fr.xl_tag), fr.seqno)) ekf_raise(fr, EKF_ST_STALE_JAC);
}

template <typename T, int NU, int MODEL, int NB, bool QPREV>
__device__ __forceinline__ void fr_role_chunk(const EkfFrame& fr, int chunk, double* sm) {
    constexpr int RD = EkfModel<MODEL>::RD, LMD = EkfModel<MODEL>::LMD, JC = EkfModel<MODEL>::JC;
    constexpr int NWV = FR_T / 64;
    double* hs = sm;
    double* a_lds = sm + fr.k * JC;
    const bool fix = fr.wprev != nullptr;
    const size_t a_len = fr_chunk_a_len(fr.kpad, fix, (int)sizeof(T));
    int* lmc = reinterpret_cast<int*>(a_lds + a_len);
    int* flag = lmc + 64;
    double* pshare = reinterpret_cast<double*>(lmc + 72);
    unsigned long long* smask_l = reinterpret_cast<unsigned long long*>(pshare + 8 * 64);
    int* nidx = reinterpret_cast<int*>(smask_l + 64);
    const int tid = threadIdx.x, m = fr.m;
    const int chunk0 = chunk * 64, cl = tid & 63, c = chunk0 + cl, g = tid >> 6;
    const T* __restrict__ P = static_cast<const T*>(fr.cov);
    const int64_t ld = fr.ld;
    if (fr.stamps && chunk == 0 && tid == 0) fr.stamps[32] = wall_clock64();
    constexpr int NJ = (16 * NB * JC + FR_T - 1) / FR_T;
    double jv[NJ], jtag = 0.0;
    const double* __restrict__ xj = fr.xl + fr.xl_jac;
    const int nel = fr.k * JC;
    auto jac_issue = [&]() {
#pragma unroll
        for (int n = 0; n < NJ; ++n) jv[n] = ekf_ldc(xj + min(tid + FR_T * n, nel - 1));
        if (tid == 0) jtag = ekf_ldc(fr.xl + fr.xl_tag);
    };
    auto jac_finish = [&]() {
        int spin = 0;
#pragma unroll
        for (int n = 0; n < NJ; ++n) {
            const int e = tid + FR_T * n;
            if (e < nel) {
                double v = jv[n];
                int it = 0;
                while (ekf_is_sent(v)) {
                    if (++it > EKF_SPIN_MAX) { spin = 1; break; }
                    ekf_poll_sleep();
                    v = ekf_ldc(xj + e);
                }
                hs[e] = v;
            }
        }
        if (spin) ekf_raise(fr, EKF_ST_TIMEOUT);
        if (fr.stamps && fr.stamps_heavy && chunk == 0 && tid == 0 && NB <= 6) fr.stamps[44] = wall_clock64();
        if (tid == 0 && fr_tag_stale(jtag, fr.seqno)) ekf_raise(fr, EKF_ST_STALE_JAC);
    };
    T pcr[EKF_CAM];
    T plr[NU][LMD];
    if (tid < m) lmc[tid] = ekf_lm_column(fr, LMD, tid, false);
    if (fr.wsup && tid >= 64 && tid < 64 + fr.next_m) {
        int ni = fr.next_idx[tid - 64];
        nidx[tid - 64] = ((unsigned)ni >= (unsigned)fr.n_lm) ? 0 : ni;
    }
    if (tid == 0) { flag[1] = 0; flag[2] = 0; }
    if (NB > 1 && tid < 16) ekf_lds_flags(pshare)[tid] = 0;
    __syncthreads();
    if (fr.wsup && tid < 64) {
        unsigned long long mk = 0ull;
        if (c >= EKF_CAM && c < fr.dims) {
            const int li = (c - EKF_CAM) / LMD;
            for (int jj = 0; jj < fr.next_m; ++jj) mk |= (unsigned long long)(nidx[jj] == li) << jj;
        }
        smask_l[tid] = mk;
    }
    if (!fix) {
#pragma unroll
        for (int a = 0; a < EKF_CAM; ++a) pcr[a] = P[a * ld + c];
#pragma unroll
        for (int u = 0; u < NU; ++u) {
            const int ju = min(g + NWV * u, m - 1);
            const int c0 = lmc[ju];
#pragma unroll
            for (int d = 0; d < LMD; ++d) plr[u][d] = P[(int64_t)(c0 + d) * ld + c];
// ... 163 lines not shown
#pragma unroll
                for (int a = 0; a < EKF_CAM; ++a) pcr[a] = (T)pl[a * 64 + cl];
            }
#pragma unroll
            for (int u = 0; u < NU; ++u) {
                const int ju = min(g + NWV * u, m - 1);
#pragma unroll
                for (int d = 0; d < LMD; ++d) {
                    const int slot = EKF_CAM + LMD * ju + d;
                    if ((slot >> 6) == round) plr[u][d] = (T)pl[(slot & 63) * 64 + cl];
                }
            }
            __syncthreads();
        }
    }
    if (!fix) jac_issue();
    jac_finish();
    __syncthreads();
    FrPre<NB> pre;
    if (fr.stamps && fr.stamps_heavy && chunk == 0 && tid == 0 && NB <= 6) fr.stamps[14] = wall_clock64();
    double pc[EKF_CAM], pld[NU][LMD];
#pragma unroll
    for (int a = 0; a < EKF_CAM; ++a) pc[a] = (double)pcr[a] + ((a == c) ? ekf_qdiag(a, fr.dims, fr.nz) : 0.0);
#pragma unroll
    for (int u = 0; u < NU; ++u) {
        const int c0 = lmc[min(g + NWV * u, m - 1)];
#pragma unroll
        for (int d = 0; d < LMD; ++d) pld[u][d] = (double)plr[u][d] + ((c0 + d == c) ? fr.nz.q_lm : 0.0);
    }
    asm volatile("" ::: "memory");
    if (g < 4) fr_panel_pre<NB, MODEL>(fr, pre, smask_l, g, chunk0 + 16 * g, tid & 63);
    if (fr.stamps && fr.stamps_heavy && chunk == 0 && tid == 0 && NB <= 6) fr.stamps[15] = wall_clock64();
    const double* __restrict__ hsr = hs;
    double* __restrict__ aw = a_lds;
#pragma unroll
    for (int u = 0; u < NU; ++u) {
        const int j = g + NWV * u;
        if (j < m) {
            const double (&pl)[LMD] = pld[u];
#pragma unroll
            for (int d = 0; d < RD; ++d) {
                const int r = RD * j + d;
                const double* __restrict__ hr = hsr + r * JC;
                double acc = 0.0;
#pragma unroll
                for (int a = 0; a < EKF_CAM; ++a) acc = __builtin_fma(hr[a], pc[a], acc);
#pragma unroll
                for (int e = 0; e < LMD; ++e) acc = __builtin_fma(hr[10 + e], pl[e], acc);
                aw[r * FR_ALD + cl] = acc;
                if (fr.wdbg) fr.amat[(int64_t)r * fr.lda + c] = acc;
            }
        }
    }
    for (int r = fr.k + g; r < fr.kpad; r += NWV) aw[r * FR_ALD + cl] = 0.0;
    __syncthreads();
    if (fr.stamps && chunk == 0 && tid == 0) fr.stamps[33] = wall_clock64();
    int spin_fail = 0;
    if (g < 4) {
        const int lane = tid & 63, col0 = chunk0 + 16 * g;
        fr_panel<T, NB, MODEL>(fr, a_lds, ekf_lds_flags(flag + 1), pshare, g, col0, lane, spin_fail, pre);
        if (spin_fail && (tid & 63) == 0) ekf_raise(fr, EKF_ST_TIMEOUT);
    } else if constexpr (NB > 1) {
        fr_panel_stage<NB>(fr, a_lds, ekf_lds_flags(pshare), g - 4, tid & 63);
    }
    if (MODEL == 0) return;
    asm volatile("s_waitcnt vmcnt(0)" ::: "memory");
    __syncthreads();
    if (tid == 0) {
        const unsigned long long old =
            __hip_atomic_fetch_add(fr.done_ctr, 1ull, __ATOMIC_ACQ_REL, __HIP_MEMORY_SCOPE_AGENT);
        flag[0] = (old + 1 == fr.done_target);
    }
    __syncthreads();
    if (!flag[0]) return;
    const int blocks = fr.frozen ? 0 : fr.n_lm;
    for (int i = tid; i <= blocks; i += FR_T) {
        const int c0 = (i == 0) ? 0 : EKF_CAM + 10 * (i - 1);
        double* st = fr.state + c0;
        const double* dx = fr.dxvec + c0;
        double q[4] = {st[3], st[4], st[5], st[6]};
        const double err[3] = {ekf_ldc(dx + 7), ekf_ldc(dx + 8), ekf_ldc(dx + 9)};
        ekf_quat_inject(q, err, 1);
        const double x0 = st[0] + ekf_ldc(dx + 0), x1 = st[1] + ekf_ldc(dx + 1), x2 = st[2] + ekf_ldc(dx + 2);
        st[0] = x0; st[1] = x1; st[2] = x2;
        for (int e = 0; e < 4; ++e) st[3 + e] = q[e];
        if (fr.state_host) {
            double* sh = fr.state_host + c0;
            sh[0] = x0; sh[1] = x1; sh[2] = x2;
            for (int e = 0; e < 4; ++e) sh[3 + e] = q[e];
            if (i == 0)
                for (int e = 0; e < 3; ++e) sh[7 + e] = 0.0;
        }
        if (i == 0) {
            for (int e = 0; e < 3; ++e) st[7 + e] = 0.0;
            if (fr.traj_row) {
                fr.traj_row[0] = x0; fr.traj_row[1] = x1; fr.traj_row[2] = x2;
                for (int e = 0; e < 4; ++e) fr.traj_row[3 + e] = q[e];
            }
        }
    }
}

template <typename T, int NU, int MODEL, int NB, bool ROWS, bool QPREV>
__global__ __launch_bounds__(FR_T) void ekf_front_kernel(EkfFrame fr) {
    extern __shared__ __attribute__((aligned(16))) double fr_sm[];
    const int nb = fr.kpad / EKF_RB, nS = nb * (nb + 1) / 2;
    const int bx = blockIdx.x;
    if (bx == 0) fr_role_measure<MODEL>(fr, fr_sm);
    else if (bx <= nS) fr_role_sblock<T, MODEL, NB, ROWS, QPREV>(fr, bx - 1, nS, fr_sm);
    else if (bx == nS + 1) fr_role_factor<NB>(fr, fr_sm);
    else fr_role_chunk<T, NU, MODEL, NB, QPREV>(fr, bx - nS - 2, fr_sm);
}

template <typename T, int NU, int MODEL, int NB, bool ROWS, bool QPREV>
static void ekf_front_go_rows(const EkfFrame& fr, hipStream_t s) {
    constexpr int LMD = EkfModel<MODEL>::LMD, JC = EkfModel<MODEL>::JC;
    constexpr int NSLOT = EKF_CAM + LMD * EkfModel<MODEL>::NDET16;
    static bool once = false;
    if (!once) {
        (void)hipFuncSetAttribute(reinterpret_cast<const void*>(ekf_front_kernel<T, NU, MODEL, NB, ROWS, QPREV>),
                                  hipFuncAttributeMaxDynamicSharedMemorySize, 160 * 1024);
        once = true;
    }
    const int nb = fr.kpad / EKF_RB, nS = nb * (nb + 1) / 2;
    const bool fix = fr.wprev != nullptr;
    const size_t dots_b = sizeof(T) == 4 ? (size_t)(32 * ((NSLOT + 31) / 32)) * (32 * ((NSLOT + 31) / 32)) * 4
                                         : (size_t)(16 * ((NSLOT + 15) / 16)) * (16 * ((NSLOT + 15) / 16)) * 8;
    const size_t lds_s = ((size_t)fr.k * JC + NSLOT * 16 + 32 + fr.kpad) * 8 + 16 + (fix ? dots_b : 0);
    const size_t lds_c = ((size_t)fr.k * JC + fr_chunk_a_len(fr.kpad, fix, (int)sizeof(T))) * 8 + 72 * 4 + 8 * 64 * 8 + 64 * 8 + 64 * 4 + 16;
    const size_t lds_f = (size_t)sv_lds_doubles_any(NB) * 8;
    size_t lds = lds_s > lds_c ? lds_s : lds_c;
    if (lds_f > lds) lds = lds_f;
    if ((size_t)fr.lds_min > lds) lds = (size_t)fr.lds_min;
    hipLaunchKernelGGL((ekf_front_kernel<T, NU, MODEL, NB, ROWS, QPREV>), dim3(nS + 2 + fr.ncols / 64), dim3(FR_T), lds, s, fr);
}

template <typename T, int NU, int MODEL, int NB>
static void ekf_front_go(const EkfFrame& fr, hipStream_t s) {
    const bool qprev = fr.wprev && (fr.qprev_cam != fr.nz.q_cam || fr.qprev_err != fr.nz.q_err || fr.qprev_lm != fr.nz.q_lm);
    if (qprev) ekf_front_go_rows<T, NU, MODEL, NB, true, true>(fr, s);
    else if (fr.rrow) ekf_front_go_rows<T, NU, MODEL, NB, true, false>(fr, s);
    else ekf_front_go_rows<T, NU, MODEL, NB, false, false>(fr, s);
}

template <typename T>
void ekf_launch_front(const EkfFrame& fr, hipStream_t s) {
    const int nb = fr.kpad / EKF_RB;
#define FR_GO(NU, MODEL, NB) case NB: return ekf_front_go<T, NU, MODEL, NB>(fr, s);
    if (fr.model == 1) {
        switch (nb) {
            FR_GO(4, 1, 1) FR_GO(4, 1, 2) FR_GO(4, 1, 3) FR_GO(4, 1, 4) FR_GO(4, 1, 5) FR_GO(4, 1, 6)
            FR_GO(4, 1, 7) FR_GO(4, 1, 8) FR_GO(4, 1, 9) FR_GO(4, 1, 10) FR_GO(4, 1, 11)
            default: return ekf_front_go<T, 4, 1, 12>(fr, s);
        }
    }
    if (fr.m <= 32) {
        switch (nb) {
            FR_GO(4, 0, 1) FR_GO(4, 0, 2) FR_GO(4, 0, 3) FR_GO(4, 0, 4) FR_GO(4, 0, 5)
            default: return ekf_front_go<T, 4, 0, 6>(fr, s);
        }
    }
    switch (nb) {
        FR_GO(8, 0, 7) FR_GO(8, 0, 8) FR_GO(8, 0, 9) FR_GO(8, 0, 10) FR_GO(8, 0, 11)
        default: return ekf_front_go<T, 8, 0, 12>(fr, s);
    }
#undef FR_GO
}
```

aruco_slam_amd/csrc/ekf_kernels.h:

```cpp
#pragma once
#include <hip/hip_runtime.h>
#include <stdint.h>
#include "ekf_device.h"

#define EKF_ST_NOT_SPD 1
#define EKF_ST_TIMEOUT 4
#define EKF_ST_STALE_JAC 16
#define EKF_ST_STALE_COL 32
#define EKF_ST_STALE_S 64
#define EKF_ST_BAD_INDEX 128
#define EKF_ST_GATE_TIMEOUT 256

struct EkfFrame {
    void* cov;
    int64_t ld;
    double* state;
    int32_t model;
    int32_t dims;
    int32_t ncols;
    int32_t m;
    int32_t k;
    int32_t kpad;
    const int32_t* idx;
    const double* z;
    double* jac;
    double* resid;
    int32_t* lmcol;
    double* amat;
    int64_t lda;
    double* sblk;
    const double* rrow;
    double* lmat;
    int32_t ldl;
    double* dinv;
    double* lop;
    double* dop;
    double* yvec;
    void* wpanel;
    int64_t ldw;
    double* wdbg;
    int32_t* status;
    double* traj_row;
    double* dxvec;
    long long* stamps;
    int32_t stamps_heavy;
    const int32_t* next_idx;
    int32_t next_m;
    void* cov_out;
    const void* wprev;
    const void* wsup_prev;
    unsigned long long* la_sync;
    unsigned long long la_signal, la_gate;
    unsigned long long cov_signal;
    long long* gate_log;
    int32_t lds_min;
    void* wsup;
    int32_t wsup_ld;
    EkfNoise nz;
    int32_t quat_mode;
    double* xl;
    double* xl_next;
    int32_t xl_dop, xl_y, xl_jac;
    int32_t xl_len;
    double* xs;
    double* xr;
    double* xs_tag;
    int32_t n_lm;
    unsigned long long* done_ctr;
    unsigned long long done_target;
    int32_t xl_tag;
    double seqno;
    double* state_host;
    int32_t* status_host;
    const uint32_t* cov_tiles;
    int32_t cov_grid;
    double qprev_cam, qprev_err, qprev_lm;
    int32_t frozen;
};

__device__ __forceinline__ double ekf_qdiag_prev(const EkfFrame& fr, int i) {
    return ekf_qdiag(i, fr.dims, EkfNoise{fr.qprev_cam, fr.qprev_err, fr.qprev_lm, 0.0});
}

__device__ __forceinline__ double ekf_row_noise(const EkfFrame& fr, int r) { return fr.rrow ? fr.rrow[r] : fr.nz.r_unc; }

__device__ __forceinline__ void ekf_raise(const EkfFrame& fr, int bits) {
    atomicOr(fr.status, bits);
    if (fr.status_host) __hip_atomic_store(fr.status_host, 1, __ATOMIC_RELAXED, __HIP_MEMORY_SCOPE_SYSTEM);
}

#define EKF_COV_SHARDS 8
#define EKF_SYNC_SHARD(s) (32 + 32 * (s))
#define EKF_SYNC_WORDS EKF_SYNC_SHARD(EKF_COV_SHARDS + 1)
#define EKF_GATE_LOG_FRAMES 2048
__device__ __forceinline__ bool ekf_cov_count(unsigned long long* ctr, unsigned long long full) {
    if (__hip_atomic_fetch_add(ctr, 1ull, __ATOMIC_RELAXED, __HIP_MEMORY_SCOPE_AGENT) + 1 != full) return false;
    __hip_atomic_store(ctr, 0ull, __ATOMIC_RELAXED, __HIP_MEMORY_SCOPE_AGENT);
    return true;
}
__device__ __forceinline__ void ekf_cov_arrive(const EkfFrame& fr) {
    asm volatile("s_waitcnt vmcnt(0)" ::: "memory");
    __builtin_amdgcn_s_barrier();
    if (threadIdx.x == 0) {
        const unsigned grid = gridDim.x, sh = blockIdx.x % EKF_COV_SHARDS;
        const unsigned in_shard = (grid + EKF_COV_SHARDS - 1 - sh) / EKF_COV_SHARDS;
        const unsigned shards = grid < EKF_COV_SHARDS ? grid : EKF_COV_SHARDS;
        if (ekf_cov_count(fr.la_sync + EKF_SYNC_SHARD(sh), in_shard) &&
            ekf_cov_count(fr.la_sync + EKF_SYNC_SHARD(EKF_COV_SHARDS), shards))
            __hip_atomic_store(fr.la_sync + 1, fr.cov_signal, __ATOMIC_RELAXED, __HIP_MEMORY_SCOPE_SYSTEM);
    }
}

__device__ __forceinline__ int ekf_lm_column(const EkfFrame& fr, int lmd, int j, bool flag) {
    int i = fr.idx[j];
    if ((unsigned)i >= (unsigned)fr.n_lm) {
        if (flag) ekf_raise(fr, EKF_ST_BAD_INDEX);
        i = 0;
    }
    return EKF_CAM + lmd * i;
}

__device__ inline void ekf_inject_camera(const EkfFrame& fr, const double err[3], const double x[3]) {
    double q[4] = {fr.state[3], fr.state[4], fr.state[5], fr.state[6]};
    ekf_quat_inject(q, err, fr.quat_mode);
    for (int i = 0; i < 4; ++i) fr.state[3 + i] = q[i];
    for (int i = 0; i < 3; ++i) fr.state[7 + i] = 0.0;
    if (fr.traj_row) {
        fr.traj_row[0] = x[0]; fr.traj_row[1] = x[1]; fr.traj_row[2] = x[2];
        for (int i = 0; i < 4; ++i) fr.traj_row[3 + i] = q[i];
    }
}

template <typename T> void ekf_launch_front(const EkfFrame& fr, hipStream_t s);
template <typename T> void ekf_launch_gather(const EkfFrame& fr, hipStream_t s);
void ekf_launch_solve(const EkfFrame& fr, hipStream_t s);
template <typename T> void ekf_launch_panel(const EkfFrame& fr, hipStream_t s);
template <typename T> void ekf_launch_cov_update(const EkfFrame& fr, int variant, hipStream_t s,
                                                 hipEvent_t e0 = nullptr, hipEvent_t e1 = nullptr);
#define EKF_STRIP_THREADS 256
template <typename T> bool ekf_launch_cov_strip(const EkfFrame& fr, int variant, hipStream_t s, hipEvent_t e0 = nullptr,
                                                hipEvent_t e1 = nullptr);
void ekf_launch_cov_update_macro(const EkfFrame& fr, hipStream_t s, hipEvent_t e0 = nullptr, hipEvent_t e1 = nullptr);
int ekf_cov_macro_table(int T, int S, uint32_t* out, int capacity);
void ekf_launch_gate(unsigned long long* counter, unsigned long long target, int32_t* status, hipStream_t s,
                     int max_polls = 1 << 22);
void ekf_launch_signal(unsigned long long* counter, unsigned long long value, hipStream_t s);

#define EKF_WIDE_REUSE_ROWS 384
#define EKF_WIDE_BLOCK 64
template <typename T> void ekf_launch_wide_front(const EkfFrame& fr, double* aw, int rp, hipStream_t s);
void ekf_launch_wide_factor(const EkfFrame& fr, double* aw, double* xinv, int rp, hipStream_t s);
template <typename T> void ekf_launch_wide_finish(const EkfFrame& fr, const double* aw, hipStream_t s);

template <typename T>
void ekf_launch_add_markers(void* cov, int64_t ld, double* state, int32_t dims,
                            const double* xyz_dev, const double* unc_dev, double default_unc,
                            int32_t count, hipStream_t s);
void ekf_launch_inject_rot(const EkfFrame& fr, int n_lm, hipStream_t s);
template <typename T>
void ekf_launch_add_markers_rot(void* cov, int64_t ld, double* state, int32_t dims, const double* pose6_dev,
                                const double* unc_dev, double default_unc, int32_t count, hipStream_t s);
void ekf_launch_log_prepare(const double* poses_dev, int64_t count, int rd, double* z_dev, hipStream_t s);
template <typename T>
void ekf_launch_log_add_markers(int model, void* cov, int64_t ld, double* state, int32_t dims, const double* poses_dev,
                                const int32_t* slots_dev, double default_unc, int32_t count, hipStream_t s);
void ekf_launch_log_fill_rows(double* traj_dev, const int32_t* pairs, int32_t count, const double* state, hipStream_t s);
#define EKF_GATE_THREADS 256
struct EkfGateArgs {
    const void* cov;
    int64_t ld;
    const double* state;
    int32_t n_lm, dims, m;
    const int32_t* idx;
    const double* z;
    const uint8_t* exempt;
    EkfNoise nz;
    double gate;
    double* mahal;
    double* mahal_host;
    int32_t* out_idx;
    double* out_z;
    const double* rows;
    double* out_rows;
    int32_t* status;
    int32_t* status_host;
    int32_t* result_host;
};
template <typename T> void ekf_launch_frame_gate(int model, const EkfGateArgs& a, hipStream_t s);
#define EKF_MOTION_THREADS 256
struct EkfMotionArgs {
    void* cov;
    int64_t ld;
    double* state;
    int32_t dims;
    double u[6];
    const int32_t* status;
};
template <typename T> void ekf_launch_motion(const EkfMotionArgs& a, hipStream_t s);
template <typename T>
void ekf_launch_cov_diag(const void* cov, int64_t ld, double* out_dev, int32_t count, hipStream_t s);

#define EKF_SMOOTH_RESIDENT_DIMS 160
#define EKF_SMOOTH_THREADS 512
struct EkfSmoothRec {
    int64_t off;
    int32_t dims;
    int32_t moved;
    double u[6];
    double q[3];
    int32_t frame0, frame1;
};
void ekf_launch_history_pack(const double* cov, int64_t ld, const double* state, int32_t dims, double* record, hipStream_t s);
void ekf_launch_smooth_rows(const double* src, double* smoothed, int32_t f0, int32_t f1, hipStream_t s);
hipError_t ekf_launch_smooth_resident(const double* history, const EkfSmoothRec* table_dev, int32_t records, int32_t nmax,
                                      int32_t lead_frames, double* smoothed, int32_t* status, hipStream_t s);
struct EkfSmoothBlocked {
    const double* history;
    EkfSmoothRec rec, next;
    double *M, *xs, *xp, *yv, *wv, *cv, *xinv;
    double* smoothed;
    int32_t* status;
};
void ekf_launch_smooth_blocked_step(const EkfSmoothBlocked& a, hipStream_t s);

#define EKF_BATCH_MAX_LANDMARKS 82
#define EKF_BATCH_MAX_VISIBLE 16
#define EKF_BATCH_ROT_MAX_LANDMARKS 24
#define EKF_BATCH_ROT_MAX_VISIBLE 8
#define EKF_BATCH_ST_NUMERIC (-5)
// ... 54 lines not shown
```

aruco_slam_amd/hip_backend.py:

```python
from __future__ import annotations

import ctypes as C
from pathlib import Path

import numpy as np

from ._build import LIB_PATH

EKF_COV_F64, EKF_COV_F32 = 0, 1
EKF_QUAT_AS_WRITTEN, EKF_QUAT_SCALAR_FIRST = 0, 1
EKF_FLAG_WIDE_FRAMES = 8
EKF_FLAG_BATCH_LARGE_MAPS = 16
EKF_FLAG_BATCH_WIDE_FRAMES = 32
EKF_FLAG_GATE = 64
EKF_FLAG_ROW_NOISE = 128
EKF_FLAG_FRAME_SCALE = 256
EKF_FLAG_MOTION = 512
EKF_COVK_AUTO, EKF_COVK_VALU, EKF_COVK_MFMA, EKF_COVK_MFMA_TILE, EKF_COVK_MFMA_MACRO = 0, 1, 2, 3, 4

GATE_LOG_FRAMES = 2048

EXPORTED_SYMBOLS = (
    "ekf_default_config", "ekf_query_sizes", "ekf_create", "ekf_destroy", "ekf_bind_buffers",
    "ekf_reset", "ekf_grow", "ekf_add_markers", "ekf_observe", "ekf_observe_device",
    "ekf_observe_sequence_device", "ekf_last_sequence_mode", "ekf_get_camera", "ekf_get_state", "ekf_get_cov_diag",
    "ekf_get_cov", "ekf_set_state", "ekf_set_cov", "ekf_num_landmarks", "ekf_sync",
    "ekf_set_fused", "ekf_set_kernel_timing", "ekf_get_kernel_timing", "ekf_debug_fetch",
    "ekf_estimate_poses_device", "ekf_estimate_poses", "ekf_last_error_string",
    "ekf_log_workspace_bytes", "ekf_observe_log", "ekf_last_log_stats",
    "ekf_batch_query_sizes", "ekf_batch_create", "ekf_batch_bind_buffers", "ekf_batch_destroy", "ekf_batch_set_noise",
    "ekf_batch_reset", "ekf_batch_set_member", "ekf_batch_get_member", "ekf_batch_num_landmarks", "ekf_batch_status",
    "ekf_batch_log_workspace_bytes", "ekf_batch_observe_logs", "ekf_batch_observe_logs_diag", "ekf_batch_replica_poses",
    "ekf_batch_replica_workspace_bytes", "ekf_batch_observe_replicas",
    "ekf_batch_set_gate", "ekf_batch_observe_logs_gated", "ekf_batch_observe_replicas_gated",
    "ekf_batch_replica_corners", "ekf_batch_observe_corner_replicas",
    "ekf_set_gate", "ekf_observe_gated", "ekf_observe_log_gated", "ekf_last_gate_stats",
    "ekf_remove_workspace_bytes", "ekf_remove_markers", "ekf_batch_remove_workspace_bytes", "ekf_batch_remove_markers",
    "ekf_observe_rows", "ekf_observe_sequence_device_rows", "ekf_observe_log_rows", "ekf_batch_observe_logs_rows",
    "ekf_advance", "ekf_get_pending_scale", "ekf_set_pending_scale", "ekf_observe_scaled",
    "ekf_observe_sequence_device_scaled", "ekf_observe_log_scaled", "ekf_batch_observe_logs_scaled",
    "ekf_batch_get_pending_scale", "ekf_batch_set_pending_scale",
    "ekf_move", "ekf_observe_moved", "ekf_observe_sequence_device_moved", "ekf_observe_log_moved",
    "ekf_batch_observe_logs_moved",
    "ekf_set_map_frozen", "ekf_get_map_frozen",
    "ekf_batch_set_map_frozen", "ekf_batch_get_map_frozen",
    "ekf_observe_log_recorded", "ekf_history_record_bytes", "ekf_history_bytes", "ekf_history_info", "ekf_history_record",
    "ekf_smooth_workspace_bytes", "ekf_smooth_history",
)


class EkfConfig(C.Structure):
    _fields_ = [
        ("max_landmarks", C.c_int32), ("max_visible", C.c_int32), ("cov_dtype", C.c_int32),
        ("quat_mode", C.c_int32), ("cov_kernel", C.c_int32), ("model", C.c_int32), ("reserved", C.c_int32), ("flags", C.c_int32),
        ("initial_camera_uncertainty", C.c_double), ("initial_landmark_uncertainty", C.c_double),
        ("r_uncertainty", C.c_double), ("q_cam", C.c_double), ("q_err", C.c_double),
        ("q_lm", C.c_double), ("stream", C.c_void_p),
    ]


class EkfError(RuntimeError):
    def __init__(self, code, msg):
        super().__init__(f"ekf_slam_hip error {code}: {msg}")
        self.code = code


_lib = None


def load_library(path: str | Path | None = None):
    global _lib
    if _lib is not None and path is None:
        return _lib
    p = Path(path) if path else LIB_PATH
    if not p.exists():
        raise FileNotFoundError(
            f"{p} not found: build it with `python -c 'import __graft_entry__ as g; g.build()'` "
            "(there is no CPU fallback for the EKF update path)")
    import torch
    lib = C.CDLL(str(p))
    dp, ip, vp = C.POINTER(C.c_double), C.POINTER(C.c_int32), C.c_void_p
    sig = {
        "ekf_default_config": [C.POINTER(EkfConfig)],
        "ekf_query_sizes": [C.POINTER(EkfConfig), C.POINTER(C.c_int64), C.POINTER(C.c_size_t),
                            C.POINTER(C.c_size_t), C.POINTER(C.c_size_t)],
        "ekf_create": [C.POINTER(EkfConfig), C.POINTER(vp)],
        "ekf_destroy": [vp],
        "ekf_bind_buffers": [vp, vp, C.c_int64, vp, vp, C.c_size_t],
        "ekf_reset": [vp, dp],
        "ekf_grow": [vp, C.c_int32, C.c_int32, vp, C.c_int64, vp, vp, C.c_size_t],
        "ekf_add_markers": [vp, dp, dp, C.c_int32],
        "ekf_observe": [vp, ip, dp, C.c_int32],
        "ekf_observe_device": [vp, vp, vp, C.c_int32],
        "ekf_observe_sequence_device": [vp, vp, vp, C.c_int32, C.c_int32, vp],
        "ekf_get_camera": [vp, dp],
        "ekf_get_state": [vp, dp, C.c_int32],
        "ekf_get_cov_diag": [vp, dp, C.c_int32],
        "ekf_get_cov": [vp, dp, C.c_int32],
        "ekf_set_state": [vp, dp, C.c_int32],
        "ekf_set_cov": [vp, dp, C.c_int32],
        "ekf_num_landmarks": [vp],
        "ekf_last_sequence_mode": [vp],
        "ekf_sync": [vp],
        "ekf_set_fused": [vp, C.c_int32],
        "ekf_set_kernel_timing": [vp, C.c_int32],
        "ekf_get_kernel_timing": [vp, C.c_int32, dp, C.POINTER(C.c_int64)],
        "ekf_debug_fetch": [vp, C.c_int32, dp, C.c_size_t],
        "ekf_estimate_poses_device": [vp, C.c_int32, C.c_double, dp, dp, C.c_int32, vp, vp],
        "ekf_estimate_poses": [dp, C.c_int32, C.c_double, dp, dp, C.c_int32, dp, vp],
        "ekf_log_workspace_bytes": [vp, C.c_int64, C.POINTER(C.c_size_t)],
        "ekf_observe_log": [vp, ip, C.POINTER(C.c_int64), C.c_int32, vp, vp, C.c_size_t, vp],
        "ekf_last_log_stats": [vp, C.POINTER(C.c_int64)],
        "ekf_set_gate": [vp, C.c_double],
        "ekf_observe_gated": [vp, ip, dp, C.c_int32, C.POINTER(C.c_uint8), dp, ip],
        "ekf_observe_log_gated": [vp, ip, C.POINTER(C.c_int64), C.c_int32, vp, vp, C.c_size_t, vp, vp],
        "ekf_last_gate_stats": [vp, C.POINTER(C.c_int64)],
        "ekf_observe_rows": [vp, ip, dp, dp, C.c_int32, C.POINTER(C.c_uint8), dp, ip],
        "ekf_observe_sequence_device_rows": [vp, vp, vp, vp, C.c_int32, C.c_int32, vp],
        "ekf_observe_log_rows": [vp, ip, C.POINTER(C.c_int64), C.c_int32, vp, vp, vp, C.c_size_t, vp, vp],
        "ekf_batch_observe_logs_rows": [vp, ip, C.POINTER(C.c_int64), C.POINTER(C.c_int64), vp, vp, vp, C.c_size_t, vp, vp,
                                        vp, vp],
        "ekf_advance": [vp, C.c_double],
        "ekf_get_pending_scale": [vp, dp],
        "ekf_set_pending_scale": [vp, C.c_double],
        "ekf_observe_scaled": [vp, ip, dp, dp, C.c_int32, C.POINTER(C.c_uint8), dp, ip, C.c_double],
        "ekf_observe_sequence_device_scaled": [vp, vp, vp, vp, dp, C.c_int32, C.c_int32, vp],
        "ekf_observe_log_scaled": [vp, ip, C.POINTER(C.c_int64), C.c_int32, vp, vp, dp, vp, C.c_size_t, vp, vp],
        "ekf_batch_observe_logs_scaled": [vp, ip, C.POINTER(C.c_int64), C.POINTER(C.c_int64), vp, vp, vp, vp, C.c_size_t, vp,
                                          vp, vp, vp],
        "ekf_batch_get_pending_scale": [vp, C.c_int32, dp],
        "ekf_batch_set_pending_scale": [vp, C.c_int32, dp],
        "ekf_move": [vp, dp],
        "ekf_observe_moved": [vp, ip, dp, dp, C.c_int32, C.POINTER(C.c_uint8), dp, ip, C.c_double, dp],
        "ekf_observe_sequence_device_moved": [vp, vp, vp, vp, dp, dp, C.c_int32, C.c_int32, vp],
        "ekf_observe_log_moved": [vp, ip, C.POINTER(C.c_int64), C.c_int32, vp, vp, dp, dp, vp, C.c_size_t, vp, vp],
        "ekf_batch_observe_logs_moved": [vp, ip, C.POINTER(C.c_int64), C.POINTER(C.c_int64), vp, vp, vp, vp, vp, C.c_size_t,
                                         vp, vp, vp, vp],
        "ekf_set_map_frozen": [vp, C.c_int32],
        "ekf_get_map_frozen": [vp],
        "ekf_batch_set_map_frozen": [vp, ip],
        "ekf_batch_get_map_frozen": [vp, ip],
        "ekf_observe_log_recorded": [vp, ip, C.POINTER(C.c_int64), C.c_int32, vp, vp, dp, dp, vp, C.c_size_t, vp, vp, vp,
                                     C.c_size_t],
        "ekf_history_record_bytes": [C.c_int32, C.POINTER(C.c_size_t)],
        "ekf_history_bytes": [vp, ip, C.POINTER(C.c_int64), C.c_int32, C.POINTER(C.c_size_t)],
        "ekf_history_info": [vp, ip, C.c_int32, ip, ip, dp, dp, ip, ip],
        "ekf_history_record": [vp, vp, C.c_int32, dp, dp, C.c_int32],
        "ekf_smooth_workspace_bytes": [vp, C.POINTER(C.c_size_t)],
        "ekf_smooth_history": [vp, vp, C.c_size_t, vp, C.c_size_t, C.c_int32, vp],
        "ekf_remove_workspace_bytes": [vp, C.c_int32, C.POINTER(C.c_size_t)],
        "ekf_remove_markers": [vp, ip, C.c_int32, vp, C.c_int64, vp, vp, C.c_size_t],
        "ekf_batch_remove_workspace_bytes": [vp, C.c_int64, C.POINTER(C.c_size_t)],
        "ekf_batch_remove_markers": [vp, ip, C.POINTER(C.c_int64), vp, C.c_int64, vp, vp, C.c_size_t],
        "ekf_batch_query_sizes": [C.POINTER(EkfConfig), C.c_int32, C.POINTER(C.c_int64), C.POINTER(C.c_size_t),
                                  C.POINTER(C.c_size_t), C.POINTER(C.c_size_t)],
        "ekf_batch_create": [C.POINTER(EkfConfig), C.c_int32, C.POINTER(vp)],
        "ekf_batch_bind_buffers": [vp, vp, C.c_int64, vp, vp, C.c_size_t],
        "ekf_batch_destroy": [vp],
        "ekf_batch_set_noise": [vp, dp],
        "ekf_batch_reset": [vp, C.c_int32, dp],
        "ekf_batch_set_member": [vp, C.c_int32, dp, C.c_int32, dp],
        "ekf_batch_get_member": [vp, C.c_int32, dp, C.c_int32, dp, C.c_int32],
        "ekf_batch_num_landmarks": [vp, ip],
        "ekf_batch_status": [vp, ip],
        "ekf_batch_log_workspace_bytes": [vp, C.c_int64, C.c_int64, C.POINTER(C.c_size_t)],
        "ekf_batch_observe_logs": [vp, ip, C.POINTER(C.c_int64), C.POINTER(C.c_int64), vp, vp, C.c_size_t, vp],
        "ekf_batch_observe_logs_diag": [vp, ip, C.POINTER(C.c_int64), C.POINTER(C.c_int64), vp, vp, C.c_size_t, vp, vp,
                                        vp],
        "ekf_batch_replica_poses": [vp, C.c_int64, dp, C.c_int32, C.c_uint64, C.c_uint32, vp, vp],
        "ekf_batch_replica_workspace_bytes": [vp, C.c_int64, C.c_int64, C.POINTER(C.c_size_t)],
        "ekf_batch_observe_replicas": [vp, ip, C.POINTER(C.c_int64), C.c_int64, vp, dp, C.c_uint64, C.c_uint32, vp,
                                       C.c_size_t, vp, vp, vp],
        "ekf_batch_set_gate": [vp, dp],
        "ekf_batch_observe_logs_gated": [vp, ip, C.POINTER(C.c_int64), C.POINTER(C.c_int64), vp, vp, C.c_size_t, vp, vp,
                                         vp, vp],
        "ekf_batch_observe_replicas_gated": [vp, ip, C.POINTER(C.c_int64), C.c_int64, vp, dp, C.c_uint64, C.c_uint32, vp,
                                             C.c_size_t, vp, vp, vp, vp],
        "ekf_batch_replica_corners": [vp, C.c_int64, dp, C.c_int32, C.c_uint64, C.c_uint32, C.c_double, dp, dp, C.c_int32,
                                      vp, vp, vp, vp],
        "ekf_batch_observe_corner_replicas": [vp, ip, C.POINTER(C.c_int64), C.c_int64, vp, dp, C.c_uint64, C.c_uint32,
                                              C.c_double, dp, dp, C.c_int32, vp, C.c_size_t, vp, vp, vp, vp, vp],
    }
    for name, args in sig.items():
        fn = getattr(lib, name)
        fn.argtypes = args
# ... 427 lines not shown
            else:
                poses_t = torch.from_numpy(poses).to(self.device, non_blocking=False)
            ws = torch.empty((nbytes.value,), dtype=torch.uint8, device=self.device)
            if traj is not None:
                traj.record_stream(self.stream)
            if mahal is not None:
                mahal.record_stream(self.stream)
            rows_t = torch.from_numpy(rows).to(self.device, non_blocking=False) if rows is not None else None
            args = (self.h, idx.ctypes.data_as(C.POINTER(C.c_int32)), offs.ctypes.data_as(C.POINTER(C.c_int64)), frames,
                    poses_t.data_ptr() if idx.shape[0] else None,
                    rows_t.data_ptr() if rows_t is not None and idx.shape[0] else None,
                    _dptr(scale) if scale is not None and frames else None,
                    _dptr(motion) if motion is not None and frames else None, ws.data_ptr(), nbytes.value,
                    traj.data_ptr() if traj is not None else None,
                    mahal.data_ptr() if mahal is not None and idx.shape[0] else None)
            if history is None:
                self._check(self.lib.ekf_observe_log_moved(*args))
            else:
                assert history.is_cuda and history.dtype == torch.uint8 and history.is_contiguous()
                history.record_stream(self.stream)
                self._check(self.lib.ekf_observe_log_recorded(*args, history.data_ptr(), history.numel()))
                self._history_frames = frames
        self._log_keep = (poses_t, ws, rows_t)
        m = np.diff(offs)
        if m.size and m.max() > 0:
            self._last_m = int(m[m > 0][-1])

    def history_bytes(self, lm_index, offsets) -> int:
        idx = np.ascontiguousarray(lm_index, dtype=np.int32).reshape(-1)
        offs = np.ascontiguousarray(offsets, dtype=np.int64).reshape(-1)
        out = C.c_size_t()
        self._check(self.lib.ekf_history_bytes(self.h, idx.ctypes.data_as(C.POINTER(C.c_int32)),
                                               offs.ctypes.data_as(C.POINTER(C.c_int64)), offs.shape[0] - 1, C.byref(out)))
        return out.value

    def new_history(self, lm_index, offsets):
        torch = self._torch
        with torch.cuda.device(self.device), torch.cuda.stream(self.stream):
            return torch.empty((self.history_bytes(lm_index, offsets),), dtype=torch.uint8, device=self.device)

    def history_info(self) -> dict:
        count = C.c_int32()
        self._check(self.lib.ekf_history_info(self.h, C.byref(count), 0, None, None, None, None, None, None))
        r = count.value
        frame, dims, stepped = (np.zeros(max(r, 1), dtype=np.int32) for _ in range(3))
        s_eff, motion = np.zeros(max(r, 1)), np.zeros((max(r, 1), 6))
        frec = np.zeros(max(self._history_frames, 1), dtype=np.int32)
        ip = C.POINTER(C.c_int32)
        self._check(self.lib.ekf_history_info(self.h, C.byref(count), max(r, 1), frame.ctypes.data_as(ip), dims.ctypes.data_as(ip),
                                              _dptr(s_eff), _dptr(motion), stepped.ctypes.data_as(ip), frec.ctypes.data_as(ip)))
        return {"frame": frame[:r], "dims": dims[:r], "s_eff": s_eff[:r], "motion": motion[:r], "stepped": stepped[:r].astype(bool),
                "frame_record": frec[:self._history_frames]}

    def history_record(self, history, r: int, dims: int):
        state, cov = np.empty(dims), np.empty((dims, dims))
        self._check(self.lib.ekf_history_record(self.h, history.data_ptr(), int(r), _dptr(state), _dptr(cov), int(dims)))
        return state, cov

    def smooth_history(self, history, frames: int, blocked: bool = False):
        torch = self._torch
        nbytes = C.c_size_t()
        self._check(self.lib.ekf_smooth_workspace_bytes(self.h, C.byref(nbytes)))
        with torch.cuda.device(self.device), torch.cuda.stream(self.stream):
            ws = torch.empty((nbytes.value,), dtype=torch.uint8, device=self.device)
            out = torch.empty((frames, 7), dtype=torch.float64, device=self.device)
            history.record_stream(self.stream)
            self._check(self.lib.ekf_smooth_history(self.h, history.data_ptr(), history.numel(), ws.data_ptr(), nbytes.value,
                                                    int(bool(blocked)), out.data_ptr() if frames else None))
        return out

    LOG_STATS = ("frames_stepped", "frames_pipelined", "pipelined_runs", "markers_added")

    def last_log_stats(self) -> dict:
        out = (C.c_int64 * 4)()
        self._check(self.lib.ekf_last_log_stats(self.h, out))
        return dict(zip(self.LOG_STATS, (int(v) for v in out)))

    SEQUENCE_MODES = {0: "none", 1: "serial", 2: "pipelined", 3: "serial (the two streams share one hardware queue)",
                      4: "serial (another handle of the process is pipelining)"}

    def last_sequence_mode(self) -> str:
        return self.SEQUENCE_MODES[self.lib.ekf_last_sequence_mode(self.h)]

    def sync(self):
        self._check(self.lib.ekf_sync(self.h))

    def get_state(self, count=None):
        n = self.dims if count is None else count
        out = np.empty(n)
        self._check(self.lib.ekf_get_state(self.h, _dptr(out), n))
        return out

    def get_cov_diag(self):
        out = np.empty(self.dims)
        self._check(self.lib.ekf_get_cov_diag(self.h, _dptr(out), self.dims))
        return out

    def get_cov(self):
        n = self.dims
        out = np.empty((n, n))
        self._check(self.lib.ekf_get_cov(self.h, _dptr(out), n))
        return out

    def set_state_cov(self, state, cov):
        state = np.ascontiguousarray(state, dtype=np.float64)
        n_lm = (state.shape[0] - 10) // self.lm_dims
        if n_lm > self.max_landmarks:
            self.grow(n_lm)
        self._check(self.lib.ekf_set_state(self.h, _dptr(state), n_lm))
        cov = np.ascontiguousarray(cov, dtype=np.float64)
        assert cov.shape == (state.shape[0], state.shape[0])
        self._check(self.lib.ekf_set_cov(self.h, _dptr(cov), state.shape[0]))

    def set_kernel_timing(self, enable):
        self._check(self.lib.ekf_set_kernel_timing(self.h, int(enable)))

    def kernel_timing(self):
        out = {}
        for i, name in enumerate(self.KERNEL_NAMES):
            us, cnt = C.c_double(), C.c_int64()
            self._check(self.lib.ekf_get_kernel_timing(self.h, i, C.byref(us), C.byref(cnt)))
            out[name] = (us.value, cnt.value)
        if self.fused:
            out = {"front": out["gather"], "cov_update": out["cov_update"]}
        return out

    def set_fused(self, enable: bool):
        self._check(self.lib.ekf_set_fused(self.h, int(bool(enable))))
        if enable:
            self.cfg.flags &= ~4
        else:
            self.cfg.flags |= 4
        self.fused = bool(enable)

    def debug_enable_w(self):
        dummy = np.zeros(1)
        self._check(self.lib.ekf_debug_fetch(self.h, -1, _dptr(dummy), 1))

    def debug_enable_stamps(self, light: bool = False):
        dummy = np.zeros(1)
        self._check(self.lib.ekf_debug_fetch(self.h, -3 if light else -2, _dptr(dummy), 1))

    def debug_fetch(self, what: str, m: int):
        rd = self.rows_per_detection
        k, kp, n = rd * m, -(-rd * m // 16) * 16, self.dims
        shape = {"jac": (k, 20 if rd == 7 else 13), "resid": (k,), "L": (kp, kp), "W": (kp, n), "A": (k, n),
                 "stamps": (64,), "gate_log": (GATE_LOG_FRAMES, 4)}[what]
        code = {"jac": 0, "resid": 1, "L": 2, "W": 3, "A": 4, "stamps": 5, "gate_log": 6}[what]
        out = np.empty(shape)
        self._check(self.lib.ekf_debug_fetch(self.h, code, _dptr(out), out.size))
        return out
```

include/ekf_slam_hip.h:

```cpp
#ifndef EKF_SLAM_HIP_H
#define EKF_SLAM_HIP_H

#include <stddef.h>
#include <stdint.h>

#ifdef __cplusplus
extern "C" {
#endif

typedef struct ekf_filter ekf_filter;

enum { EKF_COV_F64 = 0, EKF_COV_F32 = 1 };
enum { EKF_QUAT_AS_WRITTEN = 0, EKF_QUAT_SCALAR_FIRST = 1 };
enum { EKF_MODEL_EKF = 0, EKF_MODEL_ROTATIONS = 1 };
enum { EKF_FLAG_WIDE_FRAMES = 8 };
enum { EKF_FLAG_BATCH_LARGE_MAPS = 16 };
enum { EKF_FLAG_BATCH_WIDE_FRAMES = 32 };
enum { EKF_FLAG_GATE = 64 };
enum { EKF_FLAG_ROW_NOISE = 128 };
enum { EKF_FLAG_FRAME_SCALE = 256 };
enum { EKF_FLAG_MOTION = 512 };
enum { EKF_COVK_AUTO = 0, EKF_COVK_VALU = 1, EKF_COVK_MFMA = 2, EKF_COVK_MFMA_TILE = 3, EKF_COVK_MFMA_MACRO = 4 };

enum {
    EKF_OK = 0,
    EKF_ERR_INVALID = -1,
    EKF_ERR_CAPACITY = -2,
    EKF_ERR_HIP = -3,
    EKF_ERR_STATE = -4,
    EKF_ERR_NUMERIC = -5
};

typedef struct ekf_config {
    int32_t max_landmarks;
    int32_t max_visible;
    int32_t cov_dtype;
    int32_t quat_mode;
    int32_t cov_kernel;
    int32_t model;
    int32_t reserved;
    int32_t flags;
    double initial_camera_uncertainty;
    double initial_landmark_uncertainty;
    double r_uncertainty;
    double q_cam;
    double q_err;
    double q_lm;
    void *stream;
} ekf_config;

int ekf_default_config(ekf_config *cfg);

int ekf_query_sizes(const ekf_config *cfg, int64_t *ld, size_t *cov_bytes,
                    size_t *state_bytes, size_t *workspace_bytes);

int ekf_create(const ekf_config *cfg, ekf_filter **out);
int ekf_destroy(ekf_filter *f);

int ekf_bind_buffers(ekf_filter *f, void *cov_dev, int64_t ld, double *state_dev,
                     void *workspace_dev, size_t workspace_bytes);

int ekf_grow(ekf_filter *f, int32_t new_max_landmarks, int32_t new_max_visible, void *cov_dev, int64_t ld,
             double *state_dev, void *workspace_dev, size_t workspace_bytes);

int ekf_reset(ekf_filter *f, const double initial_camera_pose[10]);

int ekf_add_markers(ekf_filter *f, const double *cam_frame_xyz,
                    const double *diag_uncertainty, int32_t count);

int ekf_observe(ekf_filter *f, const int32_t *lm_index, const double *z, int32_t m);
int ekf_observe_device(ekf_filter *f, const int32_t *lm_index_dev,
                       const double *z_dev, int32_t m);

int ekf_observe_sequence_device(ekf_filter *f, const int32_t *lm_index_dev,
                                const double *z_dev, int32_t m, int32_t frames,
                                double *trajectory_dev);
enum { EKF_SEQ_NONE = 0, EKF_SEQ_SERIAL = 1, EKF_SEQ_PIPELINED = 2, EKF_SEQ_SERIAL_ONE_QUEUE = 3, EKF_SEQ_SERIAL_OTHER_HANDLE = 4 };
int ekf_last_sequence_mode(const ekf_filter *f);

int ekf_log_workspace_bytes(const ekf_filter *f, int64_t detections, size_t *bytes);
int ekf_observe_log(ekf_filter *f, const int32_t *lm_index, const int64_t *offsets, int32_t frames,
                    const double *poses_dev, void *log_ws, size_t log_ws_bytes, double *trajectory_dev);
int ekf_last_log_stats(const ekf_filter *f, int64_t out[4]);

int ekf_get_camera(ekf_filter *f, double out[10]);
int ekf_get_state(ekf_filter *f, double *out, int32_t count);
int ekf_get_cov_diag(ekf_filter *f, double *out, int32_t count);
int ekf_get_cov(ekf_filter *f, double *out, int32_t dims);

int ekf_set_state(ekf_filter *f, const double *state, int32_t num_landmarks);
int ekf_set_cov(ekf_filter *f, const double *cov, int32_t dims);

int ekf_num_landmarks(const ekf_filter *f);
int ekf_sync(ekf_filter *f);

int ekf_set_fused(ekf_filter *f, int32_t enable);

int ekf_set_kernel_timing(ekf_filter *f, int32_t enable);
int ekf_get_kernel_timing(ekf_filter *f, int32_t which, double *mean_us, int64_t *launches);

int ekf_debug_fetch(ekf_filter *f, int32_t what, double *out, size_t count);

int ekf_estimate_poses_device(const double *corners_dev, int32_t count, double marker_size,
                              const double camera_matrix[9], const double *dist_coeffs, int32_t n_dist,
                              double *poses_dev, void *stream);
int ekf_estimate_poses(const double *corners, int32_t count, double marker_size,
                       const double camera_matrix[9], const double *dist_coeffs, int32_t n_dist,
                       double *poses, void *stream);

typedef struct ekf_batch ekf_batch;
int ekf_batch_query_sizes(const ekf_config *cfg, int32_t members, int64_t *ld, size_t *cov_bytes, size_t *state_bytes,
                          size_t *workspace_bytes);
int ekf_batch_create(const ekf_config *cfg, int32_t members, ekf_batch **out);
int ekf_batch_bind_buffers(ekf_batch *b, double *cov_dev, int64_t ld, double *state_dev, void *ws_dev, size_t ws_bytes);
int ekf_batch_destroy(ekf_batch *b);
int ekf_batch_set_noise(ekf_batch *b, const double *noise);
int ekf_batch_reset(ekf_batch *b, int32_t member, const double *initial_poses);
int ekf_batch_set_member(ekf_batch *b, int32_t member, const double *state, int32_t num_landmarks, const double *cov);
int ekf_batch_get_member(ekf_batch *b, int32_t member, double *state, int32_t count, double *cov , int32_t dims);
int ekf_batch_num_landmarks(const ekf_batch *b, int32_t *out );
int ekf_batch_status(ekf_batch *b, int32_t *out );
int ekf_batch_log_workspace_bytes(const ekf_batch *b, int64_t detections, int64_t frames, size_t *bytes);
int ekf_batch_observe_logs(ekf_batch *b, const int32_t *lm_index, const int64_t *frame_offsets, const int64_t *member_frames,
                           const double *poses_dev, void *log_ws, size_t log_ws_bytes, double *trajectory_dev);
int ekf_batch_observe_logs_diag(ekf_batch *b, const int32_t *lm_index, const int64_t *frame_offsets,
                                const int64_t *member_frames, const double *poses_dev, void *log_ws, size_t log_ws_bytes,
                                double *trajectory_dev, double *nis_dev, double *cam_cov_dev);

int ekf_batch_replica_poses(const double *poses_dev, int64_t detections, const double *sigma, int32_t replicas, uint64_t seed,
                            uint32_t first_replica, double *out_dev, void *stream);
int ekf_batch_replica_workspace_bytes(const ekf_batch *b, int64_t detections, int64_t frames, size_t *bytes);
int ekf_batch_observe_replicas(ekf_batch *b, const int32_t *lm_index, const int64_t *frame_offsets, int64_t frames,
                               const double *poses_dev, const double *sigma, uint64_t seed, uint32_t first_replica, void *ws,
                               size_t ws_bytes, double *trajectory_dev, double *nis_dev, double *cam_cov_dev);

int ekf_batch_set_gate(ekf_batch *b, const double *gate );
int ekf_batch_observe_logs_gated(ekf_batch *b, const int32_t *lm_index, const int64_t *frame_offsets,
                                 const int64_t *member_frames, const double *poses_dev, void *log_ws, size_t log_ws_bytes,
                                 double *trajectory_dev, double *nis_dev, double *cam_cov_dev, double *mahal_dev);
int ekf_batch_observe_replicas_gated(ekf_batch *b, const int32_t *lm_index, const int64_t *frame_offsets, int64_t frames,
                                     const double *poses_dev, const double *sigma, uint64_t seed, uint32_t first_replica,
                                     void *ws, size_t ws_bytes, double *trajectory_dev, double *nis_dev,
                                     double *cam_cov_dev, double *mahal_dev);

int ekf_batch_replica_corners(const double *corners_dev, int64_t detections, const double *sigma_px, int32_t replicas,
                              uint64_t seed, uint32_t first_replica, double marker_size, const double camera_matrix[9],
                              const double *dist_coeffs, int32_t n_dist, double *poses_dev, uint8_t *flipped_dev,
                              double *noisy_corners_dev, void *stream);
int ekf_batch_observe_corner_replicas(ekf_batch *b, const int32_t *lm_index, const int64_t *frame_offsets, int64_t frames,
                                      const double *corners_dev, const double *sigma_px, uint64_t seed,
                                      uint32_t first_replica, double marker_size, const double camera_matrix[9],
                                      const double *dist_coeffs, int32_t n_dist, void *ws, size_t ws_bytes,
                                      double *trajectory_dev, double *nis_dev, double *cam_cov_dev, double *mahal_dev,
                                      uint8_t *flipped_dev);

int ekf_set_gate(ekf_filter *f, double gate);
int ekf_observe_gated(ekf_filter *f, const int32_t *lm_index, const double *z, int32_t m, const uint8_t *exempt ,
                      double *mahal , int32_t *survivors );
int ekf_observe_log_gated(ekf_filter *f, const int32_t *lm_index, const int64_t *offsets, int32_t frames,
                          const double *poses_dev, void *log_ws, size_t log_ws_bytes, double *trajectory_dev,
                          double *mahal_dev );
// ... 90 lines not shown
```

Baseline: 42980.

## Add early-start front kernel on a third stream to overlap consecutive frames

Adds an early-start variant of the fused front kernel. It alternates between the main stream and a new third stream, gated by device-side counters, so the next frame's front can launch before the previous covariance update finishes. The front signals a release once its last y block is written and counts block completion so the covariance gate can wait on both. It is enabled only when cfg.flags bit 2 is set or the new form setter selects it, after a runtime probe that the third stream runs concurrently. It adds spin-wait gate kernels and relaxed atomic state stores, and risks deadlock or timeout if the streams share a queue.

```diff
diff --git a/aruco_slam_amd/_build.py b/aruco_slam_amd/_build.py
--- a/aruco_slam_amd/_build.py
+++ b/aruco_slam_amd/_build.py
@@ -9,7 +9,7 @@
 CSRC = PKG / "csrc"
 LIB_DIR = PKG / "lib"
 LIB_PATH = LIB_DIR / "libekf_slam_hip.so"
-SOURCES = ["ekf_api.hip", "ekf_batch_api.hip", "ekf_small_kernels.hip", "ekf_front.hip", "ekf_front_f64.hip", "ekf_cov_update.hip", "ekf_cov_macro.hip", "ekf_cov_strip.hip", "ekf_pose_ippe.hip",
+SOURCES = ["ekf_api.hip", "ekf_batch_api.hip", "ekf_small_kernels.hip", "ekf_front.hip", "ekf_front_f64.hip", "ekf_front_early.hip", "ekf_front_early_f64.hip", "ekf_cov_update.hip", "ekf_cov_macro.hip", "ekf_cov_strip.hip", "ekf_pose_ippe.hip",
            "ekf_wide.hip", "ekf_log.hip", "ekf_gate.hip", "ekf_remove.hip", "ekf_motion.hip", "ekf_batch.hip", "ekf_batch_rot.hip", "ekf_batch_wide.hip", "ekf_batch_moved.hip", "ekf_batch_wide_moved.hip",
            "ekf_batch_frozen.hip", "ekf_batch_wide_frozen.hip",
            "ekf_batch_replicas.hip", "ekf_batch_corner_replicas.hip", "ekf_smooth.hip"]
diff --git a/aruco_slam_amd/csrc/ekf_api.hip b/aruco_slam_amd/csrc/ekf_api.hip
--- a/aruco_slam_amd/csrc/ekf_api.hip
+++ b/aruco_slam_amd/csrc/ekf_api.hip
@@ -163,6 +163,7 @@
     Layout lay{};
     hipStream_t stream = nullptr;
     hipStream_t big = nullptr;
+    hipStream_t front2 = nullptr;
     hipEvent_t ev_front = nullptr;
     GetterShortcut shortcut;
     int device = 0;
@@ -180,7 +181,10 @@
     uint64_t done_total = 0;
     uint64_t la_base = 0;
     int la_ok = -1;
+    int early_ok = -1;
     int seq_mode = EKF_SEQ_NONE;
+    int seq_detail = 0;
+    int seq_form = 0;
     int tiles_T = -1, tiles_grid = 0;
     PinnedBuffer ring, readback, tiles_host;
     int slot = 0;
@@ -351,6 +355,7 @@
     if (f->tiles_T == T) return EKF_OK;
     HIP_TRY(hipStreamSynchronize(f->stream));
     HIP_TRY(hipStreamSynchronize(f->big));
+    if (f->front2) HIP_TRY(hipStreamSynchronize(f->front2));
     const int grid = ekf_cov_macro_table(T, kMacroSuper, f->tiles_host.at<uint32_t>(0), L.tiles_cap);
     if (grid <= 0) return fail(EKF_ERR_STATE, "macro-tile launch table does not fit the workspace");
     HIP_TRY(hipMemcpy(f->at<uint32_t>(L.off_tiles), f->tiles_host.get(), (size_t)grid * 4, hipMemcpyHostToDevice));
@@ -464,6 +469,7 @@
         if (state_count > 0)
             HIP_TRY(hipMemcpyAsync(f->readback.at<double>(256), f->state, (size_t)state_count * 8, hipMemcpyDeviceToHost, f->stream));
         HIP_TRY(hipStreamSynchronize(f->stream));
+        if (f->front2) HIP_TRY(hipStreamSynchronize(f->front2));
         release_pipelining_token(f);
     }
     const int32_t* info = f->readback.at<int32_t>(0);
@@ -533,22 +539,68 @@
 bool take_pipelining_token(ekf_filter* f) {
     ekf_filter* owner = nullptr;
     if (!g_pipelining.compare_exchange_strong(owner, f) && owner != f) {
-        bool idle = hipStreamQuery(owner->stream) == hipSuccess && hipStreamQuery(owner->big) == hipSuccess;
+        bool idle = hipStreamQuery(owner->stream) == hipSuccess && hipStreamQuery(owner->big) == hipSuccess &&
+                    (!owner->front2 || hipStreamQuery(owner->front2) == hipSuccess);
         (void)hipGetLastError();
         if (!(idle && g_pipelining.compare_exchange_strong(owner, f))) return false;
     }
     return true;
 }
 
+bool early_start_asked(const ekf_filter* f) { return f->seq_form == 2 || (f->seq_form == 0 && (f->cfg.flags & 2) != 0); }
+bool early_start_wanted(const ekf_filter* f, int dims, int kpad) {
+    const int nb = kpad / EKF_RB;
+    const int grid = nb * (nb + 1) / 2 + 2 + (int)round_up(dims, 128) / 64;
+    if (2 * grid > 256) return false;
+    return f->early_ok == 1 && early_start_asked(f);
+}
+
+int probe_front2(ekf_filter* f) {
+    if (f->early_ok >= 0) return EKF_OK;
+    unsigned long long* probe = f->at<unsigned long long>(f->lay.off_sync) + 2;
+    int32_t* pstat = f->at<int32_t>(f->lay.off_sync) + 8;
+    std::vector<hipStream_t> failed;
+    auto attempt = [&]() {
+        hipStream_t fresh = nullptr;
+        HIP_TRY(hipStreamCreateWithFlags(&fresh, hipStreamNonBlocking));
+        if (f->front2) failed.push_back(f->front2);
+        f->front2 = fresh;
+        for (hipStream_t other : {f->stream, f->big}) {
+            HIP_TRY(hipMemsetAsync(probe, 0, 64, f->stream));
+            HIP_TRY(hipStreamSynchronize(f->stream));
+            HIP_TRY(hipStreamSynchronize(f->big));
+            ekf_launch_gate(probe, 1ull, pstat, f->front2, 1 << 14);
+            ekf_launch_signal(probe, 1ull, other);
+            HIP_TRY(hipStreamSynchronize(f->front2));
+            HIP_TRY(hipStreamSynchronize(other));
+            int32_t ps = 0;
+            HIP_TRY(hipMemcpy(&ps, pstat, 4, hipMemcpyDeviceToHost));
+            if (ps != 0) return (int)EKF_OK;
+        }
+        f->early_ok = 1;
+        return (int)EKF_OK;
+    };
+    f->early_ok = 0;
+    int rc = EKF_OK;
+    for (int i = 0; i < 16 && f->early_ok == 0 && rc == EKF_OK; ++i) rc = attempt();
+    for (hipStream_t s : failed) {
+        (void)hipStreamSynchronize(s);
+        (void)hipStreamDestroy(s);
+    }
+    return rc;
+}
+
 int choose_pipelining(ekf_filter* f, bool want_runs, int* mode) {
     *mode = EKF_SEQ_SERIAL;
+    f->seq_detail = 0;
     if (!want_runs || f->frozen) return EKF_OK;
     int rc = probe_queues(f);
     if (rc) return rc;
     if (f->la_ok == 0) *mode = EKF_SEQ_SERIAL_ONE_QUEUE;
     else if (!take_pipelining_token(f)) *mode = EKF_SEQ_SERIAL_OTHER_HANDLE;
     else *mode = EKF_SEQ_PIPELINED;
-    return EKF_OK;
+    if (*mode == EKF_SEQ_PIPELINED && early_start_asked(f)) rc = probe_front2(f);
+    return rc;
 }
 
 struct RunFrame {
@@ -574,6 +626,15 @@
     const uint64_t base = f->la_base;
     f->shortcut.run();
     RunFrame nx = frame_at(0);
+    const bool early = early_start_wanted(f, L.lmd * f->n_lm + EKF_CAM, (int)round_up(L.rd * nx.m, EKF_RB));
+    f->seq_detail = early ? 2 : 1;
+    unsigned long long* const c_rel = sync + EKF_SYNC_REL;
+    unsigned long long* const c_done = sync + EKF_SYNC_DONE;
+    auto front_stream = [&](int t) { return (!early || ((frames - 1 - t) & 1) == 0) ? f->stream : f->front2; };
+    if (early && front_stream(0) != f->stream) {
+        ekf_launch_signal(sync + EKF_SYNC_JOIN, base + 1, f->stream);
+        ekf_launch_gate(sync + EKF_SYNC_JOIN, base + 1, status, f->front2);
+    }
     EkfNoise nz_before{};
     for (int t = 0; t < frames; ++t) {
         const int par = t & 1;
@@ -595,6 +656,11 @@
         fr.la_sync = sync;
         fr.la_signal = (t > 0) ? base + (uint64_t)t : 0;
         fr.la_gate = (t > 0) ? base + (uint64_t)t : 0;
+        if (early) {
+            fr.la_gate = (t > 1) ? base + (uint64_t)t - 1 : 0;
+            fr.cov_signal = base + (uint64_t)t + 1;
+            if (t > 0) ekf_launch_gate(c_rel, base + (uint64_t)t, status, front_stream(t));
+        }
         fr.lds_min = grid <= 100 ? 148 * 1024 : 0;
         if (t + 1 < frames) {
             nx = frame_at(t + 1);
@@ -603,15 +669,21 @@
             fr.wsup = wsup[par];
         }
         bind_exchange(f, fr);
-        by_cov_type(f, [&](auto elem) { ekf_launch_front<decltype(elem)>(fr, f->stream); });
+        by_cov_type(f, [&](auto elem) {
+            if (early) ekf_launch_front_early<decltype(elem)>(fr, front_stream(t));
+            else ekf_launch_front<decltype(elem)>(fr, f->stream);
+        });
         EkfFrame cu = fr;
+        cu.cov_signal = 0;
         cu.cov = cbuf[par];
         cu.cov_out = cbuf[par ^ 1];
         if (t + 1 < frames) {
-            ekf_launch_gate(sync, base + (uint64_t)t + 1, status, f->big);
+            if (early) ekf_launch_gate2(sync, base + (uint64_t)t + 1, c_done, base + (uint64_t)t + 1, status, f->big);
+            else ekf_launch_gate(sync, base + (uint64_t)t + 1, status, f->big);
             cu.cov_signal = base + (uint64_t)t + 1;
             by_cov_type(f, [&](auto elem) { ekf_launch_cov_update<decltype(elem)>(cu, 2, f->big); });
         } else {
+            if (early) ekf_launch_gate(sync + 1, base + (uint64_t)t, status, f->stream);
             by_cov_type(f, [&](auto elem) { ekf_launch_cov_update<decltype(elem)>(cu, 2, f->stream); });
         }
         HIP_TRY(hipGetLastError());
@@ -953,6 +1025,10 @@
         (void)hipStreamSynchronize(f->big);
         (void)hipStreamDestroy(f->big);
     }
+    if (f->front2) {
+        (void)hipStreamSynchronize(f->front2);
+        (void)hipStreamDestroy(f->front2);
+    }
     release_pipelining_token(f);
     if (f->ev_front) (void)hipEventDestroy(f->ev_front);
     if (f->ev_gate) (void)hipEventDestroy(f->ev_gate);
@@ -1004,6 +1080,7 @@
     HIP_TRY(hipSetDevice(f->device));
     HIP_TRY(hipStreamSynchronize(f->stream));
     HIP_TRY(hipStreamSynchronize(f->big));
+    if (f->front2) HIP_TRY(hipStreamSynchronize(f->front2));
     release_pipelining_token(f);
     const Layout& ol = f->lay;
     char* nws = static_cast<char*>(workspace_dev);
@@ -1092,6 +1169,8 @@
     HIP_TRY(hipSetDevice(f->device));
     const Layout& L = f->lay;
     HIP_TRY(hipStreamSynchronize(f->stream));
+    HIP_TRY(hipStreamSynchronize(f->big));
+    if (f->front2) HIP_TRY(hipStreamSynchronize(f->front2));
     int rc = clear_buffers(f, f->cov, f->state, f->ws, L);
     if (rc) return rc;
     restart_workspace(f);
@@ -1300,6 +1379,7 @@
     f->reset_gate_stats();
     if (f->gate_on() || motion || f->frozen) {
         f->seq_mode = EKF_SEQ_SERIAL;
+        f->seq_detail = 0;
         f->shortcut.log();
         for (int t = 0; t < frames; ++t) {
             int s = m;
@@ -1912,6 +1992,13 @@
 }
 
 int ekf_last_sequence_mode(const ekf_filter* f) { return f ? f->seq_mode : EKF_ERR_INVALID; }
+int ekf_last_sequence_detail(const ekf_filter* f) { return f ? f->seq_detail : EKF_ERR_INVALID; }
+int ekf_set_sequence_form(ekf_filter* f, int32_t form) {
+    if (!f) return fail(EKF_ERR_INVALID, "filter handle is NULL");
+    if (form < 0 || form > 2) return fail(EKF_ERR_INVALID, "form must be 0 (by the rule), 1 (two-stream) or 2 (early start)");
+    f->seq_form = form;
+    return EKF_OK;
+}
 
 int ekf_set_map_frozen(ekf_filter* f, int32_t frozen) {
     int rc = check_ready(f);
diff --git a/aruco_slam_amd/csrc/ekf_cov_update.hip b/aruco_slam_amd/csrc/ekf_cov_update.hip
--- a/aruco_slam_amd/csrc/ekf_cov_update.hip
+++ b/aruco_slam_amd/csrc/ekf_cov_update.hip
@@ -311,6 +311,20 @@
 __global__ void ekf_signal_kernel(unsigned long long* counter, unsigned long long value) {
     if (threadIdx.x == 0) __hip_atomic_store(counter, value, __ATOMIC_RELAXED, __HIP_MEMORY_SCOPE_SYSTEM);
 }
+__global__ void ekf_gate2_kernel(unsigned long long* counter_a, unsigned long long target_a, unsigned long long* counter_b,
+                                 unsigned long long target_b, int32_t* status, int max_polls) {
+    if (threadIdx.x != 0) return;
+    int it = 0;
+    while (__hip_atomic_load(counter_a, __ATOMIC_RELAXED, __HIP_MEMORY_SCOPE_SYSTEM) < target_a ||
+           __hip_atomic_load(counter_b, __ATOMIC_RELAXED, __HIP_MEMORY_SCOPE_SYSTEM) < target_b) {
+        if (++it > max_polls) { atomicOr(status, EKF_ST_GATE_TIMEOUT); break; }
+        __builtin_amdgcn_s_sleep(8);
+    }
+}
+void ekf_launch_gate2(unsigned long long* counter_a, unsigned long long target_a, unsigned long long* counter_b,
+                      unsigned long long target_b, int32_t* status, hipStream_t s, int max_polls) {
+    hipLaunchKernelGGL(ekf_gate2_kernel, dim3(1), dim3(64), 0, s, counter_a, target_a, counter_b, target_b, status, max_polls);
+}
 void ekf_launch_gate(unsigned long long* counter, unsigned long long target, int32_t* status, hipStream_t s, int max_polls) {
     hipLaunchKernelGGL(ekf_gate_kernel, dim3(1), dim3(64), 0, s, counter, target, status, max_polls);
 }
diff --git a/aruco_slam_amd/csrc/ekf_front_early.hip b/aruco_slam_amd/csrc/ekf_front_early.hip
--- /dev/null
+++ b/aruco_slam_amd/csrc/ekf_front_early.hip
@@ -0,0 +1,4 @@
+#define FR_EARLY 1
+#include "ekf_front_impl.h"
+
+template void ekf_launch_front_early<float>(const EkfFrame&, hipStream_t);
diff --git a/aruco_slam_amd/csrc/ekf_front_early_f64.hip b/aruco_slam_amd/csrc/ekf_front_early_f64.hip
--- /dev/null
+++ b/aruco_slam_amd/csrc/ekf_front_early_f64.hip
@@ -0,0 +1,4 @@
+#define FR_EARLY 1
+#include "ekf_front_impl.h"
+
+template void ekf_launch_front_early<double>(const EkfFrame&, hipStream_t);
diff --git a/aruco_slam_amd/csrc/ekf_front_impl.h b/aruco_slam_amd/csrc/ekf_front_impl.h
--- a/aruco_slam_amd/csrc/ekf_front_impl.h
+++ b/aruco_slam_amd/csrc/ekf_front_impl.h
@@ -1,5 +1,16 @@
 #pragma once
 #include "ekf_solve_big.h"
+
+#ifndef FR_EARLY
+#define FR_EARLY 0
+#endif
+#if FR_EARLY
+#define FR_NS fr_early_start
+#else
+#define FR_NS fr_two_stream
+#endif
+namespace FR_NS {
+constexpr bool kEarly = FR_EARLY != 0;
 
 #define FR_T 512
 #define FR_ALD 66
@@ -20,6 +31,48 @@
 typedef float fr_f32x16 __attribute__((ext_vector_type(16)));
 
 __device__ __forceinline__ void ekf_poll_sleep() { __builtin_amdgcn_s_sleep(4); }
+
+__device__ __forceinline__ void fr_st_store(const EkfFrame& fr, double* p, double v) {
+    if constexpr (kEarly) __hip_atomic_store(p, v, __ATOMIC_RELAXED, __HIP_MEMORY_SCOPE_AGENT);
+    else *p = v;
+}
+
+__device__ __forceinline__ long long* fr_early_log(const EkfFrame& fr) {
+    return fr.gate_log ? fr.gate_log + 4 * ((long long)fr.seqno & (EKF_GATE_LOG_FRAMES - 1)) : nullptr;
+}
+__device__ __forceinline__ void fr_early_enter(const EkfFrame& fr, int bx) {
+    const int tid = threadIdx.x;
+    if (tid < 64) {
+        if (tid == 0) {
+            if (bx == 0 && fr.la_signal)
+                __hip_atomic_store(fr.la_sync, fr.la_signal, __ATOMIC_RELAXED, __HIP_MEMORY_SCOPE_SYSTEM);
+            const long long t_res = (bx == 0 && fr.gate_log) ? wall_clock64() : 0;
+            int it = 0;
+            while ((fr.la_signal &&
+                    __hip_atomic_load(fr.la_sync + EKF_SYNC_DONE, __ATOMIC_RELAXED, __HIP_MEMORY_SCOPE_SYSTEM) < fr.la_signal) ||
+                   (fr.la_gate &&
+                    __hip_atomic_load(fr.la_sync + 1, __ATOMIC_RELAXED, __HIP_MEMORY_SCOPE_SYSTEM) < fr.la_gate)) {
+                if (++it > (1 << 22)) { ekf_raise(fr, EKF_ST_GATE_TIMEOUT); break; }
+                __builtin_amdgcn_s_sleep(4);
+            }
+            if (bx == 0 && fr.gate_log) {
+                long long* row = fr_early_log(fr);
+                row[0] = t_res;
+                row[1] = wall_clock64();
+            }
+        }
+        __builtin_amdgcn_fence(__ATOMIC_ACQUIRE, "agent");
+    }
+    __syncthreads();
+}
+__device__ __forceinline__ void fr_early_arrive(const EkfFrame& fr) {
+    asm volatile("s_waitcnt vmcnt(0)" ::: "memory");
+    __syncthreads();
+    if (threadIdx.x == 0 && ekf_cov_count(fr.la_sync + EKF_SYNC_DONE_CNT, gridDim.x)) {
+        __hip_atomic_store(fr.la_sync + EKF_SYNC_DONE, fr.cov_signal, __ATOMIC_RELAXED, __HIP_MEMORY_SCOPE_SYSTEM);
+        if (fr.gate_log) fr_early_log(fr)[3] = wall_clock64();
+    }
+}
 
 template <int MODEL>
 __device__ __forceinline__ void fr_measure(const EkfFrame& fr, const double* cam, const int* lmc, double* hs,
@@ -255,9 +308,9 @@
     if (fr.stamps && !fr.stamps_heavy && tid == 0) {
         const long long now = wall_clock64();
         fr.stamps[16 + ((long long)fr.seqno & 15)] = now;
-        if (fr.gate_log) fr.gate_log[4 * ((long long)fr.seqno & (EKF_GATE_LOG_FRAMES - 1))] = now;
-    }
-    if (fr.la_signal && tid == 0)
+        if (fr.gate_log && !kEarly) fr.gate_log[4 * ((long long)fr.seqno & (EKF_GATE_LOG_FRAMES - 1))] = now;
+    }
+    if (fr.la_signal && !kEarly && tid == 0)
         __hip_atomic_store(fr.la_sync, fr.la_signal, __ATOMIC_RELAXED, __HIP_MEMORY_SCOPE_SYSTEM);
     double cam[EKF_CAM];
 #pragma unroll
@@ -275,14 +328,15 @@
         ekf_stc(fr.xl + fr.xl_tag + 16, fr.seqno);
     }
     if (fr.stamps && tid == 0) fr.stamps[55] = wall_clock64();
-    if (fr.la_gate && tid == 0) {
-        const long long g0 = fr.gate_log ? wall_clock64() : 0;
+    if (!kEarly && fr.la_gate && tid == 0) {
+        const bool glog = fr.gate_log != nullptr;
+        const long long g0 = glog ? wall_clock64() : 0;
         int it = 0;
         while (__hip_atomic_load(fr.la_sync + 1, __ATOMIC_RELAXED, __HIP_MEMORY_SCOPE_SYSTEM) < fr.la_gate) {
             if (++it > (1 << 22)) { ekf_raise(fr, EKF_ST_GATE_TIMEOUT); break; }
             __builtin_amdgcn_s_sleep(8);
         }
-        if (fr.gate_log) {
+        if (glog) {
             long long* row = fr.gate_log + 4 * ((long long)fr.seqno & (EKF_GATE_LOG_FRAMES - 1));
             row[1] = g0;
             row[2] = wall_clock64();
@@ -399,6 +453,12 @@
     }
     __device__ __forceinline__ void put_y(int b, double yv, int c, bool active) {
         if (active) ekf_stc(fr.xl + fr.xl_y + EKF_RB * b + c, yv);
+        if constexpr (kEarly) {
+            if (fr.wsup && b == fr.kpad / EKF_RB - 1 && active && c == 0) {
+                __hip_atomic_store(fr.la_sync + EKF_SYNC_REL, fr.cov_signal, __ATOMIC_RELAXED, __HIP_MEMORY_SCOPE_SYSTEM);
+                if (fr.gate_log) fr_early_log(fr)[2] = wall_clock64();
+            }
+        }
     }
 };
 
@@ -752,7 +812,7 @@
         double nv = 0.0;
         if (g == 0 && (col < 3 || (col >= EKF_CAM && col < fr.dims && !fr.frozen))) {
             nv = st_old + part;
-            fr.state[col] = nv;
+            fr_st_store(fr, fr.state + col, nv);
             if (fr.state_host) fr.state_host[col] = nv;
         }
         if (col0 == 0) {
@@ -762,15 +822,15 @@
                 double qv[4] = {q_old[0], q_old[1], q_old[2], q_old[3]};
                 const double err[3] = {e0, e1, e2};
                 ekf_quat_inject_n(qv, q_rn, err, fr.quat_mode);
-                for (int i = 0; i < 4; ++i) fr.state[3 + i] = qv[i];
-                for (int i = 0; i < 3; ++i) fr.state[7 + i] = 0.0;
+                for (int i = 0; i < 4; ++i) fr_st_store(fr, fr.state + 3 + i, qv[i]);
+                for (int i = 0; i < 3; ++i) fr_st_store(fr, fr.state + 7 + i, 0.0);
                 if (fr.state_host) {
                     for (int i = 0; i < 4; ++i) fr.state_host[3 + i] = qv[i];
                     for (int i = 0; i < 3; ++i) fr.state_host[7 + i] = 0.0;
                 }
                 if (fr.traj_row) {
-                    fr.traj_row[0] = x0; fr.traj_row[1] = x1; fr.traj_row[2] = x2;
-                    for (int i = 0; i < 4; ++i) fr.traj_row[3 + i] = qv[i];
+                    fr_st_store(fr, fr.traj_row + 0, x0); fr_st_store(fr, fr.traj_row + 1, x1); fr_st_store(fr, fr.traj_row + 2, x2);
+                    for (int i = 0; i < 4; ++i) fr_st_store(fr, fr.traj_row + 3 + i, qv[i]);
                 }
             }
         }
@@ -1100,8 +1160,8 @@
         const double err[3] = {ekf_ldc(dx + 7), ekf_ldc(dx + 8), ekf_ldc(dx + 9)};
         ekf_quat_inject(q, err, 1);
         const double x0 = st[0] + ekf_ldc(dx + 0), x1 = st[1] + ekf_ldc(dx + 1), x2 = st[2] + ekf_ldc(dx + 2);
-        st[0] = x0; st[1] = x1; st[2] = x2;
-        for (int e = 0; e < 4; ++e) st[3 + e] = q[e];
+        fr_st_store(fr, st + 0, x0); fr_st_store(fr, st + 1, x1); fr_st_store(fr, st + 2, x2);
+        for (int e = 0; e < 4; ++e) fr_st_store(fr, st + 3 + e, q[e]);
         if (fr.state_host) {
             double* sh = fr.state_host + c0;
             sh[0] = x0; sh[1] = x1; sh[2] = x2;
@@ -1110,10 +1170,10 @@
                 for (int e = 0; e < 3; ++e) sh[7 + e] = 0.0;
         }
         if (i == 0) {
-            for (int e = 0; e < 3; ++e) st[7 + e] = 0.0;
+            for (int e = 0; e < 3; ++e) fr_st_store(fr, st + 7 + e, 0.0);
             if (fr.traj_row) {
-                fr.traj_row[0] = x0; fr.traj_row[1] = x1; fr.traj_row[2] = x2;
-                for (int e = 0; e < 4; ++e) fr.traj_row[3 + e] = q[e];
+                fr_st_store(fr, fr.traj_row + 0, x0); fr_st_store(fr, fr.traj_row + 1, x1); fr_st_store(fr, fr.traj_row + 2, x2);
+                for (int e = 0; e < 4; ++e) fr_st_store(fr, fr.traj_row + 3 + e, q[e]);
             }
         }
     }
@@ -1124,10 +1184,12 @@
     extern __shared__ __attribute__((aligned(16))) double fr_sm[];
     const int nb = fr.kpad / EKF_RB, nS = nb * (nb + 1) / 2;
     const int bx = blockIdx.x;
+    if constexpr (kEarly) fr_early_enter(fr, bx);
     if (bx == 0) fr_role_measure<MODEL>(fr, fr_sm);
     else if (bx <= nS) fr_role_sblock<T, MODEL, NB, ROWS, QPREV>(fr, bx - 1, nS, fr_sm);
     else if (bx == nS + 1) fr_role_factor<NB>(fr, fr_sm);
     else fr_role_chunk<T, NU, MODEL, NB, QPREV>(fr, bx - nS - 2, fr_sm);
+    if constexpr (kEarly) fr_early_arrive(fr);
 }
 
 template <typename T, int NU, int MODEL, int NB, bool ROWS, bool QPREV>
@@ -1184,3 +1246,12 @@
     }
 #undef FR_GO
 }
+}
+
+#if FR_EARLY
+template <typename T>
+void ekf_launch_front_early(const EkfFrame& fr, hipStream_t s) { FR_NS::ekf_launch_front<T>(fr, s); }
+#else
+template <typename T>
+void ekf_launch_front(const EkfFrame& fr, hipStream_t s) { FR_NS::ekf_launch_front<T>(fr, s); }
+#endif
diff --git a/aruco_slam_amd/csrc/ekf_kernels.h b/aruco_slam_amd/csrc/ekf_kernels.h
--- a/aruco_slam_amd/csrc/ekf_kernels.h
+++ b/aruco_slam_amd/csrc/ekf_kernels.h
@@ -92,6 +92,10 @@
 #define EKF_COV_SHARDS 8
 #define EKF_SYNC_SHARD(s) (32 + 32 * (s))
 #define EKF_SYNC_WORDS EKF_SYNC_SHARD(EKF_COV_SHARDS + 1)
+#define EKF_SYNC_REL 16
+#define EKF_SYNC_JOIN 20
+#define EKF_SYNC_DONE 48
+#define EKF_SYNC_DONE_CNT 80
 #define EKF_GATE_LOG_FRAMES 2048
 __device__ __forceinline__ bool ekf_cov_count(unsigned long long* ctr, unsigned long long full) {
     if (__hip_atomic_fetch_add(ctr, 1ull, __ATOMIC_RELAXED, __HIP_MEMORY_SCOPE_AGENT) + 1 != full) return false;
@@ -132,6 +136,7 @@
 }
 
 template <typename T> void ekf_launch_front(const EkfFrame& fr, hipStream_t s);
+template <typename T> void ekf_launch_front_early(const EkfFrame& fr, hipStream_t s);
 template <typename T> void ekf_launch_gather(const EkfFrame& fr, hipStream_t s);
 void ekf_launch_solve(const EkfFrame& fr, hipStream_t s);
 template <typename T> void ekf_launch_panel(const EkfFrame& fr, hipStream_t s);
@@ -145,6 +150,8 @@
 void ekf_launch_gate(unsigned long long* counter, unsigned long long target, int32_t* status, hipStream_t s,
                      int max_polls = 1 << 22);
 void ekf_launch_signal(unsigned long long* counter, unsigned long long value, hipStream_t s);
+void ekf_launch_gate2(unsigned long long* counter_a, unsigned long long target_a, unsigned long long* counter_b,
+                      unsigned long long target_b, int32_t* status, hipStream_t s, int max_polls = 1 << 22);
 
 #define EKF_WIDE_REUSE_ROWS 384
 #define EKF_WIDE_BLOCK 64
diff --git a/aruco_slam_amd/hip_backend.py b/aruco_slam_amd/hip_backend.py
--- a/aruco_slam_amd/hip_backend.py
+++ b/aruco_slam_amd/hip_backend.py
@@ -23,7 +23,8 @@
 EXPORTED_SYMBOLS = (
     "ekf_default_config", "ekf_query_sizes", "ekf_create", "ekf_destroy", "ekf_bind_buffers",
     "ekf_reset", "ekf_grow", "ekf_add_markers", "ekf_observe", "ekf_observe_device",
-    "ekf_observe_sequence_device", "ekf_last_sequence_mode", "ekf_get_camera", "ekf_get_state", "ekf_get_cov_diag",
+    "ekf_observe_sequence_device", "ekf_last_sequence_mode", "ekf_last_sequence_detail", "ekf_set_sequence_form",
+    "ekf_get_camera", "ekf_get_state", "ekf_get_cov_diag",
     "ekf_get_cov", "ekf_set_state", "ekf_set_cov", "ekf_num_landmarks", "ekf_sync",
     "ekf_set_fused", "ekf_set_kernel_timing", "ekf_get_kernel_timing", "ekf_debug_fetch",
     "ekf_estimate_poses_device", "ekf_estimate_poses", "ekf_last_error_string",
@@ -101,6 +102,8 @@
         "ekf_set_cov": [vp, dp, C.c_int32],
         "ekf_num_landmarks": [vp],
         "ekf_last_sequence_mode": [vp],
+        "ekf_last_sequence_detail": [vp],
+        "ekf_set_sequence_form": [vp, C.c_int32],
         "ekf_sync": [vp],
         "ekf_set_fused": [vp, C.c_int32],
         "ekf_set_kernel_timing": [vp, C.c_int32],
@@ -694,6 +697,14 @@
     def last_sequence_mode(self) -> str:
         return self.SEQUENCE_MODES[self.lib.ekf_last_sequence_mode(self.h)]
 
+    SEQUENCE_FORMS = {0: "serial", 1: "two-stream", 2: "early start"}
+
+    def last_sequence_detail(self) -> str:
+        return self.SEQUENCE_FORMS[self.lib.ekf_last_sequence_detail(self.h)]
+
+    def set_sequence_form(self, form: int):
+        self._check(self.lib.ekf_set_sequence_form(self.h, int(form)))
+
     def sync(self):
         self._check(self.lib.ekf_sync(self.h))
 
diff --git a/include/ekf_slam_hip.h b/include/ekf_slam_hip.h
--- a/include/ekf_slam_hip.h
+++ b/include/ekf_slam_hip.h
@@ -77,6 +77,8 @@
                                 double *trajectory_dev);
 enum { EKF_SEQ_NONE = 0, EKF_SEQ_SERIAL = 1, EKF_SEQ_PIPELINED = 2, EKF_SEQ_SERIAL_ONE_QUEUE = 3, EKF_SEQ_SERIAL_OTHER_HANDLE = 4 };
 int ekf_last_sequence_mode(const ekf_filter *f);
+int ekf_last_sequence_detail(const ekf_filter *f);
+int ekf_set_sequence_form(ekf_filter *f, int32_t form);
 
 int ekf_log_workspace_bytes(const ekf_filter *f, int64_t detections, size_t *bytes);
 int ekf_observe_log(ekf_filter *f, const int32_t *lm_index, const int64_t *offsets, int32_t frames,
```

Result: slower. 42220 (-1.8%).
